# jnsquire/sregex

Measured on AMD Instinct MI355X. Metric: GB/s input scanned (whole job), gen-data stream resident in HBM, higher is better.
Workload: dtype u8; 1 GPU; configs[1]: /[a-z]+@[a-z]+\.[a-z]+/ Pike first-match + captures; 1 stream x 4.00 GiB gen-data (abccc.. + 'aaabbccb'); bytes_per_gpu=4294967293, streams_per_gpu=1, segment_bytes=16896, fixup_rounds=0, matches=0, engine=scan, lineage_passes=0, world_size=1

## Files before the change

### sregex_amd/csrc/sre_hip_batch.cpp

```cpp
#include <sregex_hip.h>
#include "sre_hip_runtime.h"
#include "sre_hip_scan.h"
#include "sre_scan_host.h"
#include "sre_dfa.h"
#include "sre_nfa.h"
#include "sre_hip_nfa.h"
#include "sre_nfa_wide.h"
#include "sre_hip_nfa_wide.h"
#include "sre_pwave.h"
#include "sre_hip_lines.h"
#include "sre_lines_gather.h"
#include "sre_lines_route.h"
#include "sre_lines_route_key.h"
#include "sre_lines_sort.h"
#include "sre_lines_sort_text.h"
#include "sre_lines_tally.h"
#include "sre_lines_tally_top.h"
#include "sre_lines_distinct.h"
#include "sre_lines_sums.h"
#include "sre_lines_keyset.h"
#include "sre_lines_join.h"
#include "sre_hip_streams.h"
#include "sre_streams_nfa.h"
#include <stddef.h>
#include <stdio.h>
#include <stdlib.h>
#include <string.h>
#include <atomic>
#include <chrono>
#include <initializer_list>
#include <vector>

#define SRE_SPECULATIVE_FIXUPS 2

struct sre_hip_scanner_s {
    sre_program_t     *prog;
    sre_hip_program_s *dp;
    int                mode, engine;
    char               kernel_name[64];
    uint32_t           ovec_slots;
    size_t             cap_streams;
    const void       **d_ptrs;
    uint64_t          *d_lens;
    int64_t           *d_records;
    void              *d_ctx;
    size_t             ctx_stride, ctx_cap;
    uint64_t          *h_lens;
    const void       **h_ptrs;
    size_t             last_n;
    hipStream_t        last_stream;
    sre_dfa_t                *dfa;
    sre_scan_device_tables_t *tab;
    uint32_t                  seg_override;
    uint64_t                  seg_cap_env;
    sre_scan_geom_t           geom;
    uint64_t                 *d_seg_first, *h_seg_first;
    sre_seg_summary_t        *d_sum;
    sre_seg_digest_t         *d_digest;
    size_t                    sum_cap;
    sre_stream_status_t      *d_status, *h_status;
    void                     *d_acc;
    int64_t                  *d_lo, *h_lo;
    uint16_t                 *d_scratch;
    size_t                    scratch_cap;
    sre_seg_lineage_t        *d_maps, *d_blocks;
    size_t                    maps_cap;
    uint8_t                  *d_fn;
    size_t                    fn_cap;
    int                       exact_passes;
    int                       lineage_passes;
    uint32_t                  next_init_variant;
    int                       blocks_per_cu;
    hipStream_t               tail_stream;
    bool                      tail_stream_set;
    int                       fixup_rounds;
    hipEvent_t                ev0, ev1;
    int                       ev_valid;
    sre_int_t                *h_records;
    hipEvent_t                ev_done;
    uint64_t                 *d_in, *h_in;
    unsigned char            *d_out, *h_out;
    sre_nfa_t                *nfa;
    sre_nfa_tables_t          ntab;
    sre_nfa_sa_tables_t       satab;
    bool                      use_sa;
    sre_nfa_wide_t           *wnfa;
    sre_nfa_wide_tables_t     wtab;
    uint64_t                 *d_wsets;
    bool                      wide_kernel;
    struct NfaCount          *cnt;
    uint8_t                  *d_sflags, *h_sflags;
    sre_nfa_count_req_t      *d_creq, *h_creq;
    size_t                    cnt_cap;
    int                       count_rounds;
    sre_pwave_hdr_t          *h_pwave;
    void                     *d_pwave;
    size_t                    layout_n;
    sre_nfa_summary_t        *d_nsum;
    size_t                    nsum_cap;
    uint64_t                 *d_belief;
    uint8_t                  *d_bvalid;
    uint64_t                 *d_nmat;
    size_t                    nmat_cap;
    void                     *d_nacc;
    sre_nfa_status_t         *d_nstatus, *h_nstatus;
    const uint64_t           *d_eset;
    uint64_t                 *d_ends;
    size_t                    ends_cap;
    uint64_t                 *d_lblk;
    size_t                    lblk_cap;
    int64_t                  *d_rows;
    size_t                    rows_cap;
    sre_lines_info_t         *d_linfo, *h_linfo;
    bool                      last_lines;
    int                       line_batches;
    double                    lines_kernel_ms;
    bool                      lines_device;
    size_t                    short_lines;
    hipEvent_t                ev_l0, ev_l1;
    uint64_t                 *d_fval;
    size_t                    fval_cap;
    uint64_t                 *d_fblk;
    size_t                    fblk_cap;
    uint64_t                 *d_cbits;
    size_t                    cbits_cap;
    uint64_t                 *d_cblk;
    size_t                    cblk_cap;
    uint64_t                 *d_fstart;
    size_t                    fstart_cap;
    uint8_t                  *d_lit;
    uint8_t                  *h_lit;
    size_t                    lit_len;
    bool                      lit_valid;
    uint64_t                 *d_rcnt;
    size_t                    rcnt_cap;
    uint64_t                 *d_rval;
    size_t                    rval_cap;
    uint64_t                 *d_rmeta;
    size_t                    rmeta_cap;
    int32_t                  *d_rmap;
    int32_t                  *h_rmap;
    bool                      rmap_valid;
    uint64_t                 *d_rres, *h_rres;
    uint64_t                 *d_ttab;
    size_t                    ttab_cap;
    uint32_t                 *d_tslot;
    size_t                    tslot_cap;
    uint64_t                 *d_vval;
    size_t                    vval_cap;
    uint64_t                 *d_vstart;
    size_t                    vstart_cap;
    sre_ls_agg_t             *d_vcopy;
    size_t                    vcopy_cap;
    int64_t                  *d_jkey;
    size_t                    jkey_cap;
    uint64_t                 *d_kitem[2];
    size_t                    kitem_cap[2];
    int8_t                   *d_sclass;
    size_t                    sclass_cap;
    uint32_t                 *d_sline[2];
    size_t                    sline_cap[2];
    uint64_t                 *d_pcount;
    size_t                    pcount_cap;
    sre_ls_agg_t             *d_psums;
    size_t                    psums_cap;
    uint64_t                 *d_pfirst;
    size_t                    pfirst_cap;
    uint32_t                 *d_pinv;
    size_t                    pinv_cap;
    uint64_t                 *d_pstart;
    size_t                    pstart_cap;
};

struct NfaCountStream {
    const uint8_t *base;
    uint64_t       n;
    uint64_t       cur;
    uint64_t       q;
    uint64_t       horizon;
    uint32_t       var_cur, var_q, mode_q;
    int64_t        count;
    bool           done, error;
    std::vector<sre_int_t> last;
};
struct NfaCount {
    std::vector<NfaCountStream> st;
    std::vector<size_t>         active;
};

static void
scanner_release(void *data)
{
    sre_hip_scanner_t *sc = static_cast<sre_hip_scanner_t *>(data);
    delete sc->cnt;
    free(sc->h_pwave);
    if (sc->d_pwave) (void) hipFree(sc->d_pwave);
    if (sc->d_sflags) (void) hipFree(sc->d_sflags);
    if (sc->h_sflags) (void) hipHostFree(sc->h_sflags);
    if (sc->d_creq) (void) hipFree(sc->d_creq);
    if (sc->h_creq) (void) hipHostFree(sc->h_creq);
    if (sc->d_in) (void) hipFree(sc->d_in);
    if (sc->h_in) (void) hipHostFree(sc->h_in);
    if (sc->d_out) (void) hipFree(sc->d_out);
    if (sc->h_out) (void) hipHostFree(sc->h_out);
    if (sc->d_ctx) (void) hipFree(sc->d_ctx);
    if (sc->d_sum) (void) hipFree(sc->d_sum);
    if (sc->d_digest) (void) hipFree(sc->d_digest);
    if (sc->d_acc) (void) hipFree(sc->d_acc);
    if (sc->d_lo) (void) hipFree(sc->d_lo);
    if (sc->h_lo) (void) hipHostFree(sc->h_lo);
    if (sc->d_scratch) (void) hipFree(sc->d_scratch);
    if (sc->d_fn) (void) hipFree(sc->d_fn);
    if (sc->d_maps) (void) hipFree(sc->d_maps);
    if (sc->d_blocks) (void) hipFree(sc->d_blocks);
    if (sc->ev0) (void) hipEventDestroy(sc->ev0);
    if (sc->ev1) (void) hipEventDestroy(sc->ev1);
    if (sc->ev_done) (void) hipEventDestroy(sc->ev_done);
    if (sc->ev_l0) (void) hipEventDestroy(sc->ev_l0);
    if (sc->ev_l1) (void) hipEventDestroy(sc->ev_l1);
    if (sc->d_nsum) (void) hipFree(sc->d_nsum);
    if (sc->d_belief) (void) hipFree(sc->d_belief);
    if (sc->d_bvalid) (void) hipFree(sc->d_bvalid);
    if (sc->d_nmat) (void) hipFree(sc->d_nmat);
    if (sc->d_nacc) (void) hipFree(sc->d_nacc);
    if (sc->d_ends) (void) hipFree(sc->d_ends);
    if (sc->d_lblk) (void) hipFree(sc->d_lblk);
    if (sc->d_rows) (void) hipFree(sc->d_rows);
    if (sc->d_fval) (void) hipFree(sc->d_fval);
    if (sc->d_fblk) (void) hipFree(sc->d_fblk);
    if (sc->d_cbits) (void) hipFree(sc->d_cbits);
    if (sc->d_cblk) (void) hipFree(sc->d_cblk);
    if (sc->d_fstart) (void) hipFree(sc->d_fstart);
    if (sc->d_lit) (void) hipFree(sc->d_lit);
    free(sc->h_lit);
    if (sc->d_rcnt) (void) hipFree(sc->d_rcnt);
    if (sc->d_rval) (void) hipFree(sc->d_rval);
    if (sc->d_rmeta) (void) hipFree(sc->d_rmeta);
    if (sc->d_rmap) (void) hipFree(sc->d_rmap);
    free(sc->h_rmap);
    if (sc->d_rres) (void) hipFree(sc->d_rres);
    if (sc->h_rres) (void) hipHostFree(sc->h_rres);
    if (sc->d_ttab) (void) hipFree(sc->d_ttab);
    if (sc->d_tslot) (void) hipFree(sc->d_tslot);
    if (sc->d_vval) (void) hipFree(sc->d_vval);
    if (sc->d_vstart) (void) hipFree(sc->d_vstart);
    if (sc->d_vcopy) (void) hipFree(sc->d_vcopy);
    if (sc->d_jkey) (void) hipFree(sc->d_jkey);
    if (sc->d_kitem[0]) (void) hipFree(sc->d_kitem[0]);
    if (sc->d_kitem[1]) (void) hipFree(sc->d_kitem[1]);
    if (sc->d_sclass) (void) hipFree(sc->d_sclass);
    if (sc->d_sline[0]) (void) hipFree(sc->d_sline[0]);
    if (sc->d_sline[1]) (void) hipFree(sc->d_sline[1]);
    if (sc->d_pcount) (void) hipFree(sc->d_pcount);
    if (sc->d_psums) (void) hipFree(sc->d_psums);
    if (sc->d_pfirst) (void) hipFree(sc->d_pfirst);
    if (sc->d_pinv) (void) hipFree(sc->d_pinv);
    if (sc->d_pstart) (void) hipFree(sc->d_pstart);
    if (sc->d_linfo) (void) hipFree(sc->d_linfo);
    if (sc->h_linfo) (void) hipHostFree(sc->h_linfo);
    if (sc->ntab.accept) (void) hipFree(const_cast<uint64_t *>(sc->ntab.accept));
    if (sc->ntab.follow) (void) hipFree(const_cast<uint64_t *>(sc->ntab.follow));
    if (sc->ntab.expand) (void) hipFree(const_cast<uint64_t *>(sc->ntab.expand));
    if (sc->ntab.kind) (void) hipFree(const_cast<uint8_t *>(sc->ntab.kind));
    if (sc->satab.accept) (void) hipFree(const_cast<uint64_t *>(sc->satab.accept));
    if (sc->satab.lut) (void) hipFree(const_cast<uint64_t *>(sc->satab.lut));
    if (sc->satab.expand) (void) hipFree(const_cast<uint64_t *>(sc->satab.expand));
    if (sc->d_wsets) (void) hipFree(sc->d_wsets);
    if (sc->wtab.accept) (void) hipFree(const_cast<uint64_t *>(sc->wtab.accept));
    if (sc->wtab.lut) (void) hipFree(const_cast<uint64_t *>(sc->wtab.lut));
    if (sc->wtab.expand) (void) hipFree(const_cast<uint64_t *>(sc->wtab.expand));
    if (sc->wtab.kind) (void) hipFree(const_cast<uint8_t *>(sc->wtab.kind));
    sre_nfa_wide_free(sc->wnfa);
    sre_nfa_free(sc->nfa);
    sre_scan_tables_release(sc->tab);
    sre_dfa_free(sc->dfa);
    free(sc);
}

static int
nfa_upload(sre_hip_scanner_t *sc)
{
    const sre_nfa_t *n = sc->nfa;
    const uint32_t   ns = n->nslices;
    std::vector<uint64_t> fol((size_t) ns * 256, 0), exp(16 * 256, 0);
    memcpy(fol.data(), n->follow.data(), n->follow.size() * sizeof(uint64_t));
    if (n->nassert) memcpy(exp.data(), n->expand.data(), exp.size() * sizeof(uint64_t));
    uint64_t *d_acc = NULL, *d_fol = NULL, *d_exp = NULL;
    uint8_t  *d_kind = NULL;
    SRE_HIP_TRY(hipMalloc(reinterpret_cast<void **>(&d_acc), 256 * sizeof(uint64_t)));
    sc->ntab.accept = d_acc;
// ... 360 lines not shown
sre_hip_scanner_kernel_name(sre_hip_scanner_t *sc)
{
    if (sc->kernel_name[0] == 0) {
        if (sc->engine == SRE_HIP_ENGINE_SCAN) {
            snprintf(sc->kernel_name, sizeof(sc->kernel_name), "sre_k_scan<%d, %d, %s, %s>",
                     sc->mode == SRE_HIP_PIKE_COUNT ? 2 : 1, (int) sc->tab->h.class_bits,
                     sc->tab->h.wide ? "true" : "false",
                     sc->mode == SRE_HIP_PIKE_COUNT && sc->tab->h.any_fresh ? "true" : "false");
        } else if (sc->engine == SRE_HIP_ENGINE_NFA) {
            if (sc->wide_kernel) sre_nfa_wide_kernel_name(&sc->wtab, sc->kernel_name, sizeof(sc->kernel_name));
            else if (sc->use_sa) sre_nfa_sa_kernel_name(&sc->satab, sc->kernel_name, sizeof(sc->kernel_name));
            else sre_nfa_kernel_name(sc->mode == SRE_HIP_THOMPSON ? 0 : 1, sc->ntab.nslices, sc->ntab.nassert != 0,
                                     sc->kernel_name, sizeof(sc->kernel_name));
        } else {
            snprintf(sc->kernel_name, sizeof(sc->kernel_name), "%s",
                     sc->mode == SRE_HIP_THOMPSON ? (sc->dp->has_wave ? "sre_k_thompson_wave_scan" : "sre_k_thompson_scan")
                                                  : sc->d_pwave ? "sre_k_pike_scan_wave" : "sre_k_pike_scan");
        }
    }
    return sc->kernel_name;
}

extern "C" SRE_API int
sre_hip_scanner_last_lineage_passes(sre_hip_scanner_t *sc)
{
    return sc->lineage_passes;
}

extern "C" SRE_API double
sre_hip_scanner_last_kernel_ms(sre_hip_scanner_t *sc)
{
    float ms = 0.0f;
    if (sc->last_lines) return sc->lines_kernel_ms;
    if (!sc->ev_valid) return -1.0;
    if (hipEventSynchronize(sc->ev1) != hipSuccess) return -1.0;
    if (hipEventElapsedTime(&ms, sc->ev0, sc->ev1) != hipSuccess) return -1.0;
    return (double) ms;
}

extern "C" SRE_API int
sre_hip_scanner_order_after_scan(sre_hip_scanner_t *sc, void *hip_stream)
{
    if (!sc->ev_valid) return 0;
    hipError_t e = hipStreamWaitEvent(static_cast<hipStream_t>(hip_stream), sc->ev1, 0);
    return e == hipSuccess ? 0 : sre_hip_fail("hipStreamWaitEvent", e);
}

extern "C" SRE_API int
sre_hip_scanner_set_tail_stream(sre_hip_scanner_t *sc, void *hip_stream)
{
    sc->tail_stream = static_cast<hipStream_t>(hip_stream);
    sc->tail_stream_set = hip_stream != NULL;
    return 0;
}

extern "C" SRE_API size_t
sre_hip_scanner_last_segment_bytes(sre_hip_scanner_t *sc)
{
    return sc->engine != SRE_HIP_ENGINE_VM ? sc->geom.seg_bytes : 0;
}

static size_t
record_bytes(const sre_hip_scanner_t *sc, size_t n)
{
    return n * (2 + (size_t) sc->ovec_slots) * sizeof(int64_t);
}

static int
scanner_reserve(sre_hip_scanner_t *sc, size_t n)
{
    if (n > sc->cap_streams) {
        if (sc->d_in) (void) hipFree(sc->d_in);
        if (sc->h_in) (void) hipHostFree(sc->h_in);
        if (sc->d_out) (void) hipFree(sc->d_out);
        if (sc->h_out) (void) hipHostFree(sc->h_out);
        if (sc->d_acc) (void) hipFree(sc->d_acc);
        if (sc->d_lo) (void) hipFree(sc->d_lo);
        if (sc->h_lo) (void) hipHostFree(sc->h_lo);
        sc->d_in = sc->h_in = NULL;
        sc->d_out = sc->h_out = NULL;
        sc->d_acc = NULL;
        sc->d_lo = sc->h_lo = NULL;
        sc->cap_streams = 0;
        const size_t in_bytes = (3 * n + 1) * sizeof(uint64_t);
        const size_t out_bytes = record_bytes(sc, n) + n * sizeof(sre_stream_status_t);
        static_assert(sizeof(sre_nfa_status_t) <= sizeof(sre_stream_status_t), "status block");
        static_assert(sizeof(sre_nfa_status_t) == sizeof(sre_nfa_window_t), "window layout");
        SRE_HIP_TRY(hipMalloc(reinterpret_cast<void **>(&sc->d_in), in_bytes));
        SRE_HIP_TRY(hipHostMalloc(reinterpret_cast<void **>(&sc->h_in), in_bytes, 0));
        SRE_HIP_TRY(hipMalloc(reinterpret_cast<void **>(&sc->d_out), out_bytes));
        SRE_HIP_TRY(hipHostMalloc(reinterpret_cast<void **>(&sc->h_out), out_bytes, 0));
        SRE_HIP_TRY(hipMalloc(&sc->d_acc, sre_scan_verify_acc_bytes((uint32_t) n)));
        SRE_HIP_TRY(sre_scan_verify_acc_init(sc->d_acc, (uint32_t) n, NULL));
        if (sc->engine == SRE_HIP_ENGINE_NFA) {
            if (sc->d_nacc) (void) hipFree(sc->d_nacc);
            sc->d_nacc = NULL;
            SRE_HIP_TRY(hipMalloc(&sc->d_nacc, sre_nfa_verify_acc_bytes((uint32_t) n)));
            SRE_HIP_TRY(sre_nfa_verify_acc_init(sc->d_nacc, (uint32_t) n, NULL));
        }
        SRE_HIP_TRY(hipStreamSynchronize(NULL));
        SRE_HIP_TRY(hipMalloc(reinterpret_cast<void **>(&sc->d_lo), n * sizeof(int64_t)));
        SRE_HIP_TRY(hipHostMalloc(reinterpret_cast<void **>(&sc->h_lo), n * sizeof(int64_t), 0));
        sc->cap_streams = n;
    }
    sc->layout_n = n;
    sc->h_ptrs = reinterpret_cast<const void **>(sc->h_in);
    sc->h_lens = sc->h_in + n;
    sc->h_seg_first = sc->h_in + 2 * n;
    sc->d_ptrs = reinterpret_cast<const void **>(sc->d_in);
    sc->d_lens = sc->d_in + n;
    sc->d_seg_first = sc->d_in + 2 * n;
    sc->d_records = reinterpret_cast<sre_int_t *>(sc->d_out);
    sc->h_records = reinterpret_cast<sre_int_t *>(sc->h_out);
    sc->d_status = reinterpret_cast<sre_stream_status_t *>(sc->d_out + record_bytes(sc, n));
    sc->h_status = reinterpret_cast<sre_stream_status_t *>(sc->h_out + record_bytes(sc, n));
    sc->d_nstatus = reinterpret_cast<sre_nfa_status_t *>(sc->d_status);
    sc->h_nstatus = reinterpret_cast<sre_nfa_status_t *>(sc->h_status);
    if ((sc->engine == SRE_HIP_ENGINE_VM || (sc->engine == SRE_HIP_ENGINE_NFA && sc->mode != SRE_HIP_THOMPSON && sc->d_pwave == NULL))
        && n * sc->ctx_stride > sc->ctx_cap)
    {
        if (sc->d_ctx) (void) hipFree(sc->d_ctx);
        sc->d_ctx = NULL;
        sc->ctx_cap = 0;
        SRE_HIP_TRY(hipMalloc(&sc->d_ctx, n * sc->ctx_stride));
        sc->ctx_cap = n * sc->ctx_stride;
    }
    return 0;
hip_failed:
    return -1;
}

static uint64_t
scan_seg_knobs(sre_hip_scanner_t *sc)
{
    uint64_t seg = sc->seg_override;
    const char *e = getenv("SRE_HIP_SEG_BYTES");
    if (seg == 0 && e && atoi(e) > 0 && atoi(e) % 256 == 0) seg = (uint64_t) atoi(e);
    e = getenv("SRE_HIP_SEG_CAP");
    sc->seg_cap_env = e && atoi(e) > 0 ? (uint64_t) atoi(e) : 0;
    return seg;
}

static uint64_t
nfa_seg_knobs(sre_hip_scanner_t *sc)
{
    uint64_t seg = scan_seg_knobs(sc);
    const char *e = getenv("SRE_HIP_SEG_BYTES");
    if (seg == 0 && e && atoi(e) > 0 && atoi(e) % 64 == 0) seg = (uint64_t) atoi(e);
    return seg;
}

static uint64_t
scan_seg_cap(const sre_hip_scanner_t *sc)
{
    return sc->seg_cap_env ? sc->seg_cap_env : 40960;
}

static int
scan_events(sre_hip_scanner_t *sc)
{
    if (sc->ev0 == NULL) {
        SRE_HIP_TRY(hipEventCreate(&sc->ev0));
        SRE_HIP_TRY(hipEventCreate(&sc->ev1));
    }
    return 0;
hip_failed:
    return -1;
}

static void
call_begin(sre_hip_scanner_t *sc)
{
    sc->last_lines = false;
    sc->fixup_rounds = 0;
    sc->exact_passes = 0;
    sc->lineage_passes = 0;
    sc->ev_valid = 0;
}

static void
geom_clear(sre_hip_scanner_t *sc)
{
    sc->geom = sre_scan_geom_t();
    sc->d_eset = NULL;
}

static void
geom_device(sre_hip_scanner_t *sc, uint64_t n, uint64_t seg, uint64_t nsegs)
{
    geom_clear(sc);
    sc->geom.streams = reinterpret_cast<const uint8_t *const *>(sc->d_ptrs);
    sc->geom.lens = sc->d_lens;
    sc->geom.seg_first = sc->d_seg_first;
    sc->geom.nstreams = (uint32_t) n;
    sc->geom.seg_bytes = (uint32_t) seg;
    sc->geom.nsegs = nsegs;
}

static uint64_t
scan_resident(sre_hip_scanner_t *sc)
{
    if (sc->blocks_per_cu == 0) {
        sc->blocks_per_cu = sc->engine == SRE_HIP_ENGINE_NFA
                                ? (sc->wide_kernel ? sre_nfa_wide_blocks_per_cu(&sc->wtab)
                                   : sc->use_sa ? sre_nfa_sa_blocks_per_cu(&sc->satab)
                                              : sre_nfa_blocks_per_cu(sc->mode == SRE_HIP_THOMPSON ? 0 : 1, sc->ntab.nslices,
                                                                      sc->ntab.nassert != 0))
                                                             : sre_scan_blocks_per_cu(&sc->tab->h);
    }
    return (uint64_t) sre_hip_cu_count() * (uint64_t) sc->blocks_per_cu * SRE_SCAN_BLOCK;
}

static int scan_buffers(sre_hip_scanner_t *sc, size_t nstreams, uint64_t seg, uint64_t nsegs);

static int
nfa_buffers(sre_hip_scanner_t *sc, uint64_t nsegs)
{
    if (nsegs > sc->nsum_cap) {
        if (sc->d_nsum) (void) hipFree(sc->d_nsum);
        if (sc->d_belief) (void) hipFree(sc->d_belief);
        if (sc->d_bvalid) (void) hipFree(sc->d_bvalid);
        if (sc->d_wsets) (void) hipFree(sc->d_wsets);
        sc->d_nsum = NULL;
        sc->d_belief = NULL;
        sc->d_bvalid = NULL;
        sc->d_wsets = NULL;
        sc->nsum_cap = 0;
        SRE_HIP_TRY(hipMalloc(reinterpret_cast<void **>(&sc->d_nsum), nsegs * sizeof(sre_nfa_summary_t)));
        SRE_HIP_TRY(hipMalloc(reinterpret_cast<void **>(&sc->d_belief), nsegs * nfa_words(sc) * sizeof(uint64_t)));
        if (sc->wide_kernel) SRE_HIP_TRY(hipMalloc(reinterpret_cast<void **>(&sc->d_wsets), nsegs * 2 * nfa_words(sc) * sizeof(uint64_t)));
        SRE_HIP_TRY(hipMalloc(reinterpret_cast<void **>(&sc->d_bvalid), nsegs));
        sc->nsum_cap = nsegs;
    }
    return 0;
hip_failed:
    return -1;
}

static int
scan_geometry(sre_hip_scanner_t *sc, size_t nstreams, uint32_t init_variant, uint32_t flags, uint32_t entry_state)
{
    uint64_t total = 0;
    for (size_t i = 0; i < nstreams; i++) total += sc->h_lens[i];
    uint64_t seg = scan_seg_knobs(sc);
    if (seg == 0) {
        const uint64_t resident = scan_resident(sc);
        seg = sre_scan_auto_segment(total, resident, scan_seg_cap(sc));
    }
    uint64_t nsegs = 0;
    for (size_t i = 0; i < nstreams; i++) {
        sc->h_seg_first[i] = nsegs;
        uint64_t k = (sc->h_lens[i] + seg - 1) / seg;
        nsegs += k ? k : 1;
    }
    sc->h_seg_first[nstreams] = nsegs;
    geom_clear(sc);
    sc->geom.streams = reinterpret_cast<const uint8_t *const *>(sc->d_ptrs);
    sc->geom.lens = sc->d_lens;
    sc->geom.seg_first = sc->d_seg_first;
    sc->geom.nstreams = (uint32_t) nstreams;
    sc->geom.seg_bytes = (uint32_t) seg;
    sc->geom.nsegs = nsegs;
    sc->geom.init_variant = init_variant;
    sc->geom.entry_state = entry_state;
    sc->geom.one_ptr = static_cast<const uint8_t *>(sc->h_ptrs[0]);
    sc->geom.one_len = sc->h_lens[0];
    sc->geom.flags = flags | ((nstreams == 1 && sc->engine == SRE_HIP_ENGINE_SCAN) ? SRE_GEOM_ONE : 0u);

    if (sc->engine == SRE_HIP_ENGINE_NFA) return nfa_buffers(sc, nsegs);
    return scan_buffers(sc, nstreams, seg, nsegs);
}

static int
scan_buffers(sre_hip_scanner_t *sc, size_t nstreams, uint64_t seg, uint64_t nsegs)
{
    if (nsegs > sc->sum_cap) {
        if (sc->d_sum) (void) hipFree(sc->d_sum);
        sc->d_sum = NULL;
        sc->sum_cap = 0;
        SRE_HIP_TRY(hipMalloc(reinterpret_cast<void **>(&sc->d_sum), nsegs * sizeof(sre_seg_summary_t)));
        sc->sum_cap = nsegs;
    }
    sc->geom.digest = NULL;
    if (nsegs <= SRE_VERIFY_ONE_SEGS && sc->mode != SRE_HIP_PIKE_COUNT) {
        if (sc->d_digest == NULL
            && hipMalloc(reinterpret_cast<void **>(&sc->d_digest), SRE_VERIFY_ONE_SEGS * sizeof(sre_seg_digest_t)) != hipSuccess)
        {
            sc->d_digest = NULL;
        }
        sc->geom.digest = sc->d_digest;
    }
    {
        size_t need = nstreams * ((size_t) seg + 16);
        if (need > sc->scratch_cap) {
            if (sc->d_scratch) (void) hipFree(sc->d_scratch);
            sc->d_scratch = NULL;
            sc->scratch_cap = 0;
            SRE_HIP_TRY(hipMalloc(reinterpret_cast<void **>(&sc->d_scratch), need * sizeof(uint16_t)));
            sc->scratch_cap = need;
        }
    }
    return 0;
hip_failed:
    return -1;
}

static int
nfa_windows(sre_hip_scanner_t *sc, const int64_t *d_lo, const sre_nfa_count_req_t *d_creq, hipStream_t stream)
{
    const uint32_t n = sc->geom.nstreams;
    if (sc->d_pwave) {
        SRE_HIP_TRY(sre_launch_pike_window_wave(sc->d_pwave, sc->h_pwave, sc->d_ptrs, sc->d_lens, n, sc->d_records,
                                                sc->ovec_slots, reinterpret_cast<sre_nfa_window_t *>(sc->d_nstatus), d_lo,
                                                d_creq, stream));
    } else {
        SRE_HIP_TRY(sre_launch_pike_window(sc->dp->d_blob, sc->dp->blob_bytes, sc->d_ptrs, sc->d_lens, n, sc->d_ctx, sc->ctx_stride,
                                           sc->d_records, sc->ovec_slots,
                                           reinterpret_cast<sre_nfa_window_t *>(sc->d_nstatus), d_lo,
                                           d_creq, stream));
    }
    return 0;
hip_failed:
    return -1;
}

static int
nfa_finish(sre_hip_scanner_t *sc, const int64_t *d_lo, const sre_nfa_count_req_t *d_creq, hipStream_t stream)
{
    const int kmode = sc->mode == SRE_HIP_THOMPSON ? SRE_HIP_THOMPSON : SRE_HIP_PIKE_FIRST;
    if (sc->wide_kernel) {
        SRE_HIP_TRY(sre_launch_nfa_wide_verify(kmode, sc->wtab.W, sc->geom, sc->d_nsum, sc->d_wsets, sc->d_nacc, sc->d_nstatus,
                                               sc->d_belief, sc->d_bvalid, sc->d_records, sc->ovec_slots, d_lo, stream));
    } else {
        SRE_HIP_TRY(sre_launch_nfa_verify(kmode, sc->geom, sc->d_nsum, sc->d_nacc, sc->d_nstatus,
                                          sc->d_belief, sc->d_bvalid, sc->d_records, sc->ovec_slots, d_lo, stream));
    }
    if (sc->mode != SRE_HIP_THOMPSON) return nfa_windows(sc, d_lo, d_creq, stream);
    return 0;
hip_failed:
    return -1;
}

static uint64_t
count_horizon(uint64_t dflt)
{
    const char *e = getenv("SRE_HIP_COUNT_HORIZON");
    return e && atoll(e) > 0 ? (uint64_t) atoll(e) : dflt;
}

static int
nfa_enqueue_pass(sre_hip_scanner_t *sc, size_t nstreams, uint32_t init_variant, const uint8_t *d_sflags,
                 const sre_nfa_count_req_t *d_creq, hipStream_t stream)
{
    if (scan_geometry(sc, nstreams, init_variant, 0, 0) != 0) return -1;
    sc->geom.sflags = d_sflags;
    SRE_HIP_TRY(hipMemcpyAsync(sc->d_in, sc->h_in, (3 * sc->layout_n + 1) * sizeof(uint64_t),
                               hipMemcpyHostToDevice, stream));
    if (scan_events(sc) != 0) return -1;
    {
        const bool timed = !sc->ev_valid;
        if (timed) SRE_HIP_TRY(hipEventRecord(sc->ev0, stream));
        SRE_HIP_TRY(nfa_launch_scan(sc, NULL, NULL, NULL, stream));
        if (timed) SRE_HIP_TRY(hipEventRecord(sc->ev1, stream));
        sc->ev_valid = 1;
    }
    if (sc->tail_stream_set && sc->tail_stream != stream) {
        SRE_HIP_TRY(hipStreamWaitEvent(sc->tail_stream, sc->ev1, 0));
        stream = sc->tail_stream;
    }
    return nfa_finish(sc, NULL, d_creq, stream);
hip_failed:
    return -1;
}
// ... 142 lines not shown
        SRE_HIP_TRY(hipMemcpyAsync(sc->h_out, sc->d_out, record_bytes(sc, sc->layout_n) + sc->layout_n * sizeof(sre_stream_status_t),
                                   hipMemcpyDeviceToHost, stream));
        SRE_HIP_TRY(hipStreamSynchronize(stream));
        {
            bool settled = true;
            if (nfa_settle(sc, na, sc->d_creq, stream, &settled) != 0) goto hip_failed;
            if (!settled) {
                SRE_HIP_TRY(hipMemcpyAsync(sc->h_out, sc->d_out, record_bytes(sc, sc->layout_n) + sc->layout_n * sizeof(sre_stream_status_t),
                                           hipMemcpyDeviceToHost, stream));
                SRE_HIP_TRY(hipStreamSynchronize(stream));
            }
        }
        for (size_t j = 0; j < na; j++) {
            NfaCountStream         &t = c.st[c.active[j]];
            const sre_nfa_status_t &w = sc->h_nstatus[j];
            const sre_int_t        *rec = sc->h_records + j * slots;
            const bool              truncated = (sc->h_sflags[j] & SRE_SFLAG_NO_EOF) != 0;
            if (getenv("SRE_HIP_DEBUG_COUNT")) {
                fprintf(stderr, "[sregex-hip] count round %d stream %zu: cur %llu q %llu var %u/%u mode %u len %llu%s -> ev %lld clean %lld "
                                "cmode %x rec %lld (%lld, %lld)\n", sc->count_rounds, c.active[j], (unsigned long long) t.cur,
                        (unsigned long long) t.q, t.var_cur, t.var_q, t.mode_q, (unsigned long long) sc->h_lens[j],
                        truncated ? " (truncated)" : "", (long long) w.ev_pos, (long long) w.clean_pos, w.clean_mode,
                        (long long) rec[0], (long long) rec[2], (long long) rec[3]);
            }
            if (w.ev_pos >= 0) {
                if (rec[0] < 0) {
                    fprintf(stderr, "[sregex-hip] find-all on the NFA tier: the exact window found no match behind an event\n");
                    t.error = t.done = true;
                    continue;
                }
                t.count++;
                t.last.assign(rec, rec + slots);
                const uint64_t end = (uint64_t) rec[3];
                const uint64_t gap = end > t.cur ? end - t.cur : 1;
                t.horizon = gap + gap / 4 < count_horizon(1u << 20) ? count_horizon(1u << 20) : gap + gap / 4;
                t.cur = t.q = end;
                t.var_cur = t.var_q = (w.clean_mode & SRE_NFA_MATCH_AFTER_NL) ? 1u : 2u;
                t.mode_q = 0;
                if (w.clean_mode & SRE_NFA_WINDOW_POISONED) t.error = t.done = true;
            } else if (!truncated) {
                t.done = true;
            } else if (w.clean_pos > 0) {
                t.q += (uint64_t) w.clean_pos;
                t.var_q = (w.clean_mode & SRE_NFA_CLEAN_AFTER_NL) ? 1u : 2u;
                t.mode_q = (uint32_t) (w.clean_mode & 1);
                t.horizon *= 2;
            } else {
                t.horizon *= 4;
            }
        }
    }
    sc->tail_stream_set = tail_set;
    for (size_t i = 0; i < n; i++) {
        const NfaCountStream &t = c.st[i];
        sre_int_t            *out = results + i * slots;
        if (t.count == 0) {
            out[0] = t.error ? SRE_ERROR : SRE_DECLINED;
            out[1] = 0;
            for (size_t k = 2; k < slots; k++) out[k] = -1;
        } else {
            for (size_t k = 0; k < slots; k++) out[k] = t.last[k];
            if (t.error) out[0] = SRE_ERROR;
            out[1] = (sre_int_t) t.count;
        }
    }
    return 0;
hip_failed:
    sc->tail_stream_set = tail_set;
    return -1;
}

extern "C" SRE_API int
sre_hip_scanner_last_count_rounds(sre_hip_scanner_t *sc)
{
    return sc->count_rounds;
}

extern "C" SRE_API int
sre_hip_scan_enqueue(sre_hip_scanner_t *sc, const void *const *d_streams, const size_t *lens,
    size_t nstreams, void *hip_stream)
{
    hipStream_t    stream = static_cast<hipStream_t>(hip_stream);
    const uint32_t init_variant = sc->next_init_variant;
    call_begin(sc);
    sc->next_init_variant = 0;
    if (nstreams == 0) {
        sc->last_n = 0;
        return 0;
    }
    if (scanner_reserve(sc, nstreams) != 0) return -1;
    for (size_t i = 0; i < nstreams; i++) {
        sc->h_ptrs[i] = d_streams[i];
        sc->h_lens[i] = lens[i];
    }
    if (sc->engine == SRE_HIP_ENGINE_VM) {
        SRE_HIP_TRY(hipMemcpyAsync(sc->d_in, sc->h_in, 2 * nstreams * sizeof(uint64_t),
                                   hipMemcpyHostToDevice, stream));
        if (sc->d_pwave && nstreams <= 16384) {
            SRE_HIP_TRY(sre_launch_pike_scan_wave(sc->d_pwave, sc->h_pwave, sc->mode, sc->d_ptrs, sc->d_lens,
                                                  (uint32_t) nstreams, sc->d_records, sc->ovec_slots, stream));
        } else {
            SRE_HIP_TRY(hipMemsetAsync(sc->d_ctx, 0, nstreams * sc->ctx_stride, stream));
            SRE_HIP_TRY(sre_launch_vm_scan(sc->dp->d_blob, sc->mode, sc->d_ptrs, sc->d_lens,
                                           (uint32_t) nstreams, sc->d_ctx, sc->ctx_stride,
                                           sc->d_records, sc->ovec_slots, sc->dp->has_wave, stream));
        }
    } else if (sc->engine == SRE_HIP_ENGINE_NFA && sc->cnt != NULL) {
        NfaCount &c = *sc->cnt;
        c.st.assign(nstreams, NfaCountStream());
        for (size_t i = 0; i < nstreams; i++) {
            NfaCountStream &t = c.st[i];
            t.base = static_cast<const uint8_t *>(d_streams[i]);
            t.n = lens[i];
            t.cur = t.q = 0;
            t.horizon = count_horizon(8u << 20);
            t.var_cur = t.var_q = init_variant;
            t.mode_q = 0;
            t.count = 0;
            t.done = t.error = false;
        }
        sc->count_rounds = 0;
        sc->last_n = nstreams;
        sc->last_stream = stream;
        return 0;
    } else if (sc->engine == SRE_HIP_ENGINE_NFA) {
        if (nfa_enqueue_pass(sc, nstreams, init_variant, NULL, NULL, stream) != 0) return -1;
        if (sc->tail_stream_set && sc->tail_stream != stream) stream = sc->tail_stream;
    } else {
        if (scan_geometry(sc, nstreams, init_variant, 0, 0) != 0) return -1;
        const bool one = (sc->geom.flags & SRE_GEOM_ONE) != 0;
        if (!one) {
            static const bool dma = getenv("SRE_HIP_DMA_UPLOAD") != NULL;
            if (dma) {
                SRE_HIP_TRY(hipMemcpyAsync(sc->d_in, sc->h_in, (3 * nstreams + 1) * sizeof(uint64_t),
                                           hipMemcpyHostToDevice, stream));
            } else {
                SRE_HIP_TRY(sre_launch_upload_words(sc->h_in, sc->d_in, (uint32_t) (3 * nstreams + 1), stream));
            }
        }
        if (scan_events(sc) != 0) return -1;
        SRE_HIP_TRY(hipEventRecord(sc->ev0, stream));
        SRE_HIP_TRY(sre_launch_scan(sc->tab->d_tab, sc->tab->h, sc->geom, sc->d_sum, NULL, NULL, stream));
        SRE_HIP_TRY(hipEventRecord(sc->ev1, stream));
        sc->ev_valid = 1;
        if (sc->tail_stream_set && sc->tail_stream != stream) {
            SRE_HIP_TRY(hipStreamWaitEvent(sc->tail_stream, sc->ev1, 0));
            stream = sc->tail_stream;
        }
        {
            const int fused = one && sc->geom.nsegs <= SRE_VERIFY_ONE_SEGS && sc->mode != SRE_HIP_PIKE_COUNT;
            if (!fused) SRE_HIP_TRY(sre_launch_verify(sc->tab->h, sc->geom, sc->d_sum, sc->d_acc, sc->d_status, stream));
            SRE_HIP_TRY(sre_launch_captures(sc->tab->d_tab, sc->tab->h, sc->geom, sc->d_sum, sc->d_status,
                                            sc->d_scratch, sc->d_records, sc->ovec_slots,
                                            NULL, NULL, 0, fused, stream));
        }
    }
    SRE_HIP_TRY(hipMemcpyAsync(sc->h_out, sc->d_out,
                               record_bytes(sc, nstreams)
                                   + (sc->engine != SRE_HIP_ENGINE_VM ? nstreams * sizeof(sre_stream_status_t) : 0),
                               hipMemcpyDeviceToHost, stream));
    if (sc->ev_done == NULL) SRE_HIP_TRY(hipEventCreateWithFlags(&sc->ev_done, hipEventDisableTiming));
    SRE_HIP_TRY(hipEventRecord(sc->ev_done, stream));
    sc->last_n = nstreams;
    sc->last_stream = stream;
    return 0;
hip_failed:
    return -1;
}

typedef uint64_t sre_lines_info_t::*LinfoWord;
#define LINFO(word) (&sre_lines_info_t::word)

static hipError_t
linfo_read(sre_hip_scanner_t *sc, hipStream_t stream, std::initializer_list<LinfoWord> words)
{
    const char *base = reinterpret_cast<const char *>(sc->h_linfo);
    size_t      lo = sizeof(sre_lines_info_t), hi = 0;
    for (LinfoWord w : words) {
        const size_t at = (size_t) (reinterpret_cast<const char *>(&(sc->h_linfo->*w)) - base);
        lo = at < lo ? at : lo;
        hi = at + sizeof(uint64_t) > hi ? at + sizeof(uint64_t) : hi;
    }
    return hipMemcpyAsync(reinterpret_cast<char *>(sc->h_linfo) + lo, reinterpret_cast<const char *>(sc->d_linfo) + lo, hi - lo,
                          hipMemcpyDeviceToHost, stream);
}

static int
lines_status_counters(sre_hip_scanner_t *sc, size_t n, hipStream_t stream)
{
    SRE_HIP_TRY(sre_launch_lines_settle(sc->d_status, (uint32_t) n, sc->d_linfo, stream));
    SRE_HIP_TRY(linfo_read(sc, stream, {LINFO(pending), LINFO(maps)}));
    SRE_HIP_TRY(hipStreamSynchronize(stream));
    return 0;
hip_failed:
    return -1;
}

static int
scan_settle(sre_hip_scanner_t *sc, size_t n, hipStream_t stream, bool with_captures, bool *psettled,
            bool counters = false)
{
    bool settled = true;
    int  batch = sc->mode == SRE_HIP_PIKE_COUNT ? 2 : SRE_SPECULATIVE_FIXUPS + 1;
    for (;;) {
        size_t pending = 0;
        if (counters) pending = (size_t) sc->h_linfo->pending;
        else for (size_t i = 0; i < n; i++) pending += sc->h_status[i].done ? 0 : 1;
        if (pending == 0) break;
        settled = false;
        for (int r = 0; r < batch; r++) {
            if (++sc->fixup_rounds > 1000000) {
                fprintf(stderr, "[sregex-hip] scanner fix-up did not converge\n");
                return -1;
            }
            const uint8_t *d_entry = NULL;
            static const bool count_exact = getenv("SRE_HIP_NO_COUNT_EXACT") == NULL;
            if ((sc->mode != SRE_HIP_PIKE_COUNT || count_exact) && sc->fixup_rounds > SRE_SPECULATIVE_FIXUPS) {
                if (sc->geom.nsegs > sc->fn_cap) {
                    if (sc->d_fn) (void) hipFree(sc->d_fn);
                    sc->d_fn = NULL;
                    sc->fn_cap = 0;
                    const size_t nchunks = sc->geom.nsegs / 256 + 1;
                    SRE_HIP_TRY(hipMalloc(reinterpret_cast<void **>(&sc->d_fn),
                                          sc->geom.nsegs * 64 + nchunks * 64 + nchunks + sc->geom.nsegs + 64));
                    sc->fn_cap = sc->geom.nsegs;
                }
                const size_t nchunks = sc->geom.nsegs / 256 + 1;
                uint8_t *d_comp = sc->d_fn + sc->geom.nsegs * 64, *d_chunk = d_comp + nchunks * 64;
                uint8_t *d_ent = d_chunk + nchunks;
                SRE_HIP_TRY(sre_launch_exact_entries(sc->tab->d_tab, sc->tab->h, sc->geom, sc->d_sum, sc->d_status,
                                                     sc->d_fn, d_comp, d_chunk, d_ent, stream));
                d_entry = d_ent;
                sc->exact_passes++;
            }
            SRE_HIP_TRY(sre_launch_scan(sc->tab->d_tab, sc->tab->h, sc->geom, sc->d_sum, sc->d_status, d_entry, stream));
            SRE_HIP_TRY(sre_launch_verify(sc->tab->h, sc->geom, sc->d_sum, sc->d_acc, sc->d_status, stream));
            if (with_captures) {
                SRE_HIP_TRY(sre_launch_captures(sc->tab->d_tab, sc->tab->h, sc->geom, sc->d_sum,
                                                sc->d_status, sc->d_scratch, sc->d_records,
                                                sc->ovec_slots, NULL, NULL, 0, 0, stream));
            }
        }
        if (counters) {
            if (lines_status_counters(sc, n, stream) != 0) return -1;
        } else {
            SRE_HIP_TRY(hipMemcpyAsync(sc->h_status, sc->d_status, n * sizeof(sre_stream_status_t),
                                       hipMemcpyDeviceToHost, stream));
            SRE_HIP_TRY(hipStreamSynchronize(stream));
        }
        batch = sc->mode == SRE_HIP_PIKE_COUNT ? (batch < 16 ? 2 * batch : 16) : 1;
    }
    if (psettled) *psettled = settled;
    return 0;
hip_failed:
    return -1;
}

static int
scan_lineage_pass(sre_hip_scanner_t *sc, hipStream_t stream)
{
    if (sc->geom.nsegs > sc->maps_cap) {
        if (sc->d_maps) (void) hipFree(sc->d_maps);
        if (sc->d_blocks) (void) hipFree(sc->d_blocks);
        sc->d_maps = sc->d_blocks = NULL;
        sc->maps_cap = 0;
        SRE_HIP_TRY(hipMalloc(reinterpret_cast<void **>(&sc->d_maps),
                              sc->geom.nsegs * sizeof(sre_seg_lineage_t)));
        SRE_HIP_TRY(hipMalloc(reinterpret_cast<void **>(&sc->d_blocks),
                              (sc->geom.nsegs / SRE_LINEAGE_BLOCK + 1) * sizeof(sre_seg_lineage_t)));
        sc->maps_cap = sc->geom.nsegs;
    }
    sc->lineage_passes++;
    SRE_HIP_TRY(sre_launch_lineage(sc->tab->d_tab, sc->tab->h, sc->geom, sc->d_sum,
                                   sc->d_status, sc->d_maps, sc->d_blocks, stream));
    SRE_HIP_TRY(sre_launch_captures(sc->tab->d_tab, sc->tab->h, sc->geom, sc->d_sum,
                                    sc->d_status, sc->d_scratch, sc->d_records,
                                    sc->ovec_slots, sc->d_maps, sc->d_blocks,
                                    1, 0, stream));
    return 0;
hip_failed:
    return -1;
}

extern "C" SRE_API int
sre_hip_scan_results(sre_hip_scanner_t *sc, sre_int_t *results)
{
    if (sc->last_lines) return -1;
    if (sc->last_n == 0) return 0;
    const size_t n = sc->last_n;
    hipStream_t  stream = sc->last_stream;

    const size_t bytes = n * (2 + (size_t) sc->ovec_slots) * sizeof(int64_t);
    bool         settled = true;

    if (sc->engine == SRE_HIP_ENGINE_NFA && sc->cnt != NULL) return nfa_count_rounds(sc, results);
    SRE_HIP_TRY(hipEventSynchronize(sc->ev_done));
    if (sc->engine == SRE_HIP_ENGINE_NFA && nfa_settle(sc, n, NULL, stream, &settled) != 0) return -1;
    if (sc->engine == SRE_HIP_ENGINE_SCAN) {
        if (scan_settle(sc, n, stream, true, &settled) != 0) return -1;
        if (sc->mode != SRE_HIP_THOMPSON) {
            size_t want = 0;
            for (size_t i = 0; i < n; i++) want += sc->h_status[i].need_maps != 0;
            if (want) {
                settled = false;
                if (scan_lineage_pass(sc, stream) != 0) return -1;
            }
        }
    }
    if (sc->engine == SRE_HIP_ENGINE_SCAN && getenv("SRE_HIP_DEBUG_STATUS")) {
        for (size_t i = 0; i < n && i < 8; i++) {
            const sre_stream_status_t &t = sc->h_status[i];
            fprintf(stderr, "[sregex-hip] stream %zu: rc %lld count %lld ev_pos %lld ev_sp %lld ev_state %u ev_sym %u "
                            "ev_apos %lld ev_astate %u ev_seg %lld limit %lld need_maps %d seg %u\n",
                    i, (long long) t.rc, (long long) t.count, (long long) t.ev_pos, (long long) t.ev_sp,
                    t.ev_state, t.ev_sym, (long long) t.ev_apos, t.ev_astate, (long long) t.ev_seg,
                    (long long) t.limit, t.need_maps, sc->geom.seg_bytes);
        }
        const size_t ns = sc->geom.nsegs < 16 ? (size_t) sc->geom.nsegs : 16;
        std::vector<sre_seg_summary_t> hs(ns);
// ... 159 lines not shown
    return 0;
hip_failed:
    return -1;
}

struct LinesTotals {
    int    fixups, exact, lineage;
    double kms;
    size_t nshort;
};

static int
lines_device_begin(sre_hip_scanner_t *sc, uint64_t rcap, size_t width, hipStream_t stream)
{
    if (rcap && lines_grow(&sc->d_rows, &sc->rows_cap, rcap * width * sizeof(int64_t)) != 0) return -1;
    SRE_HIP_TRY(hipMemsetAsync(&sc->d_linfo->reported, 0, sizeof(uint64_t), stream));
    return scan_events(sc);
hip_failed:
    return -1;
}

static int
lines_device_batch_end(sre_hip_scanner_t *sc, LinesTotals *tot, const LinesSink *sink, uint64_t nmax, uint64_t i0, int all,
                       uint64_t rcap, hipStream_t stream)
{
    const uint32_t slots = 2 + sc->ovec_slots;
    if (sink) {
        if (sink_select(sc, sink, slots, nmax, i0, stream) != 0) return -1;
    } else {
        SRE_HIP_TRY(sre_launch_lines_compact(sc->d_records, slots, nmax, i0, all, sc->d_ends, sc->d_lblk, sc->d_linfo, sc->d_rows,
                                             rcap, stream));
    }
    tot->fixups += sc->fixup_rounds;
    tot->exact += sc->exact_passes;
    tot->lineage += sc->lineage_passes;
    sc->line_batches++;
    return 0;
hip_failed:
    return -1;
}

static int
lines_device_end(sre_hip_scanner_t *sc, const LinesSink *sink, uint64_t n, sre_int_t *out, uint64_t rcap, size_t width,
                 uint64_t *pnrep, hipStream_t stream)
{
    if (sink) return 0;
    SRE_HIP_TRY(hipMemcpyAsync(&sc->h_linfo->reported, &sc->d_linfo->reported, sizeof(uint64_t), hipMemcpyDeviceToHost,
                               stream));
    SRE_HIP_TRY(hipStreamSynchronize(stream));
    *pnrep = n ? sc->h_linfo->reported : 0;
    {
        const uint64_t take = *pnrep < rcap ? *pnrep : rcap;
        if (take) {
            SRE_HIP_TRY(hipMemcpyAsync(out, sc->d_rows, take * width * sizeof(int64_t), hipMemcpyDeviceToHost, stream));
            SRE_HIP_TRY(hipStreamSynchronize(stream));
        }
    }
    return 0;
hip_failed:
    return -1;
}

static int
lines_scan_device(sre_hip_scanner_t *sc, const void *d_buf, uint64_t n, int all, sre_int_t *out, size_t cap,
                  uint64_t *pnrep, hipStream_t stream, LinesTotals *tot, const LinesSink *sink)
{
    const size_t   width = 3 + 2 + (size_t) sc->ovec_slots;
    const uint64_t bmax = lines_batch_limit();
    const uint64_t rcap = cap < n ? cap : n;
    const uint64_t seg_fixed = scan_seg_knobs(sc);
    const uint64_t resident = scan_resident(sc);
    if (lines_device_begin(sc, rcap, width, stream) != 0) return -1;
    for (uint64_t i0 = 0; i0 < n;) {
        const uint64_t nmax = bmax < n - i0 ? bmax : n - i0;
        if (scanner_reserve(sc, nmax) != 0) return -1;
        SRE_HIP_TRY(sre_launch_lines_geometry(d_buf, sc->d_ends, n, i0, nmax, SRE_LINES_WALK_MAX, seg_fixed, resident,
                                              scan_seg_cap(sc), reinterpret_cast<const uint8_t **>(sc->d_ptrs), sc->d_lens,
                                              sc->d_seg_first, sc->d_lblk, sc->d_linfo, stream));
        SRE_HIP_TRY(linfo_read(sc, stream, {LINFO(i1), LINFO(seg), LINFO(nsegs)}));
        SRE_HIP_TRY(hipStreamSynchronize(stream));
        const uint64_t i1 = sc->h_linfo->i1, nb = i1 - i0, seg = sc->h_linfo->seg, nsegs = sc->h_linfo->nsegs;
        call_begin(sc);
        geom_device(sc, nb, seg, nsegs);
        if (scan_buffers(sc, nb, seg, nsegs) != 0) return -1;
        SRE_HIP_TRY(hipEventRecord(sc->ev0, stream));
        SRE_HIP_TRY(sre_launch_scan(sc->tab->d_tab, sc->tab->h, sc->geom, sc->d_sum, NULL, NULL, stream));
        SRE_HIP_TRY(hipEventRecord(sc->ev1, stream));
        SRE_HIP_TRY(sre_launch_verify(sc->tab->h, sc->geom, sc->d_sum, sc->d_acc, sc->d_status, stream));
        SRE_HIP_TRY(sre_launch_captures(sc->tab->d_tab, sc->tab->h, sc->geom, sc->d_sum, sc->d_status,
                                        sc->d_scratch, sc->d_records, sc->ovec_slots, NULL, NULL, 0, 0, stream));
        if (lines_status_counters(sc, nb, stream) != 0) return -1;
        if (scan_settle(sc, nb, stream, true, NULL, true) != 0) return -1;
        if (sc->mode != SRE_HIP_THOMPSON && sc->h_linfo->maps != 0 && scan_lineage_pass(sc, stream) != 0) return -1;
        if (lines_device_batch_end(sc, tot, sink, nmax, i0, all, rcap, stream) != 0) return -1;
        {
            float ms = 0.0f;
            SRE_HIP_TRY(hipEventElapsedTime(&ms, sc->ev0, sc->ev1));
            tot->kms += ms;
        }
        i0 = i1;
    }
    return lines_device_end(sc, sink, n, out, rcap, width, pnrep, stream);
hip_failed:
    return -1;
}

static uint64_t
lines_short_max(const sre_hip_scanner_t *sc)
{
    if (sc->wide_kernel) return 0;
    const char *e = getenv("SRE_HIP_LINES_SHORT_MAX");
    if (e == NULL || *e == 0) return SRE_LINES_SHORT_MAX;
    const long long v = atoll(e);
    return v <= 0 ? 0 : v < (1ll << 20) ? (uint64_t) v : (uint64_t) 1 << 20;
}

static int
lines_scan_nfa(sre_hip_scanner_t *sc, const void *d_buf, uint64_t n, int all, sre_int_t *out, size_t cap,
               uint64_t *pnrep, hipStream_t stream, LinesTotals *tot, const LinesSink *sink)
{
    const size_t   width = 3 + 2 + (size_t) sc->ovec_slots;
    const uint64_t rcap = cap < n ? cap : n;
    const uint64_t lmax = lines_short_max(sc), short_lim = lmax ? lmax + 1 : 0;
    const uint32_t W = nfa_words(sc);
    const uint64_t seg_cost = sizeof(sre_nfa_summary_t) + W * sizeof(uint64_t) + 1 + (sc->wide_kernel ? 2 * W * sizeof(uint64_t) : 0);
    uint64_t       bmax = lines_batch_limit();
    const uint64_t seg_fixed = nfa_seg_knobs(sc);
    const uint64_t resident = scan_resident(sc);
    if (sc->mode != SRE_HIP_THOMPSON && sc->d_pwave == NULL && sc->ctx_stride) {
        const uint64_t most = SRE_LINES_NFA_WORK_MAX / sc->ctx_stride;
        if (bmax > most) bmax = most ? most : 1;
    }
    sre_lnfa_t ltab;
    memset(&ltab, 0, sizeof(ltab));
    if (short_lim) ltab = sc->use_sa ? sre_lines_nfa_tables_sa(&sc->satab) : sre_lines_nfa_tables_plain(&sc->ntab);
    if (lines_device_begin(sc, rcap, width, stream) != 0) return -1;
    if (sc->ev_l0 == NULL) {
        SRE_HIP_TRY(hipEventCreate(&sc->ev_l0));
        SRE_HIP_TRY(hipEventCreate(&sc->ev_l1));
    }
    for (uint64_t i0 = 0; i0 < n;) {
        const uint64_t nmax = bmax < n - i0 ? bmax : n - i0;
        if (scanner_reserve(sc, nmax) != 0) return -1;
        SRE_HIP_TRY(sre_launch_lines_geometry_nfa(d_buf, sc->d_ends, n, i0, nmax, short_lim, SRE_LINES_NFA_WORK_MAX, seg_cost,
                                                  seg_fixed, resident, scan_seg_cap(sc), reinterpret_cast<const uint8_t **>(sc->d_ptrs),
                                                  sc->d_lens, sc->d_seg_first, sc->d_lblk, sc->d_linfo, stream));
        SRE_HIP_TRY(linfo_read(sc, stream, {LINFO(i1), LINFO(seg), LINFO(nsegs)}));
        SRE_HIP_TRY(hipMemcpyAsync(&sc->h_linfo->nshort, &sc->d_linfo->nshort, sizeof(uint64_t), hipMemcpyDeviceToHost, stream));
        SRE_HIP_TRY(hipStreamSynchronize(stream));
        const uint64_t i1 = sc->h_linfo->i1, nb = i1 - i0, seg = sc->h_linfo->seg, nsegs = sc->h_linfo->nsegs;
        const uint64_t nshort = sc->h_linfo->nshort;
        call_begin(sc);
        geom_device(sc, nb, seg, nsegs);
        if (nsegs) {
            if (nfa_buffers(sc, nsegs) != 0) return -1;
            SRE_HIP_TRY(hipEventRecord(sc->ev0, stream));
            SRE_HIP_TRY(nfa_launch_scan(sc, NULL, NULL, NULL, stream));
            SRE_HIP_TRY(hipEventRecord(sc->ev1, stream));
            if (nfa_finish(sc, NULL, NULL, stream) != 0) return -1;
        }
        if (nshort) {
            SRE_HIP_TRY(hipEventRecord(sc->ev_l0, stream));
            SRE_HIP_TRY(sre_launch_lines_nfa(ltab, d_buf, sc->d_ends, i0, (uint32_t) nb, (uint32_t) short_lim,
                                             sc->mode == SRE_HIP_THOMPSON, sc->d_nstatus, sc->d_records, sc->ovec_slots, sc->d_lo,
                                             stream));
            SRE_HIP_TRY(hipEventRecord(sc->ev_l1, stream));
            if (sc->mode != SRE_HIP_THOMPSON && nfa_windows(sc, sc->d_lo, NULL, stream) != 0) return -1;
        }
        if (nsegs && nfa_settle_device(sc, nb, stream) != 0) return -1;
        if (lines_device_batch_end(sc, tot, sink, nmax, i0, all, rcap, stream) != 0) return -1;
        {
// ... 1438 lines not shown
            res.need_bytes = (size_t) sc->h_linfo->fneed;
            res.nwritten = (size_t) nwritten;
            res.out_bytes = (size_t) out_bytes;
            res.passes = passes;
            res.vmin = vmin;
            res.vmax = vmax;
            SRE_HIP_TRY(sre_launch_extract_gather(d_buf, d_out, sc->d_rval, sc->d_pstart, nrows * k, out_bytes, (uint32_t) delim,
                                                  (uint32_t) fsep, stream));
            const uint64_t counts_rows = counts_cap < nrows ? counts_cap : nrows, sums_rows = sums_cap < nrows ? sums_cap : nrows;
            const uint64_t index_rows = index_cap < nwritten ? index_cap : nwritten;
            SRE_HIP_TRY(sre_launch_tally_top_permute(keys, nkeys, nrows, sc->d_pcount, psums, v, sc->d_pfirst, sc->d_ends, n, sc->d_pstart,
                                                     sc->d_rval, k, sc->d_jkey, sc->d_sclass, d_counts, counts_rows, d_sums, sums_rows,
                                                     reinterpret_cast<int64_t *>(d_index), index_rows, sc->d_pinv, stream));
        }
        SRE_HIP_TRY(sre_launch_tally_top_ranks(sc->d_tslot, t.cnt, sc->d_pinv, rank_cap < n ? rank_cap : n, nkeys,
                                               reinterpret_cast<int64_t *>(d_rank), stream));
        SRE_HIP_TRY(hipStreamSynchronize(stream));
    }
    if (info) *info = res;
    return rc;
hip_failed:
    return -1;
}

extern "C" SRE_API int
sre_hip_scanner_last_line_batches(sre_hip_scanner_t *sc)
{
    return sc->line_batches;
}

extern "C" SRE_API int
sre_hip_scanner_last_lines_device(sre_hip_scanner_t *sc)
{
    return sc->lines_device ? 1 : 0;
}

extern "C" SRE_API size_t
sre_hip_scanner_last_short_lines(sre_hip_scanner_t *sc)
{
    return sc->short_lines;
}

extern "C" int
sre_hip_scan_one(sre_hip_scanner_t *sc, const void *d_buf, size_t len, int init_variant,
    sre_int_t *rec, int *poisoned, hipStream_t stream)
{
    const void *ptrs[1] = {d_buf};
    size_t      lens[1] = {len};
    sc->next_init_variant = (uint32_t) init_variant;
    if (sre_hip_scan_enqueue(sc, ptrs, lens, 1, stream) != 0) return -1;
    if (sre_hip_scan_results(sc, rec) != 0) return -1;
    if (poisoned) {
        *poisoned = sc->engine == SRE_HIP_ENGINE_SCAN ? sc->h_status[0].error
                  : sc->engine == SRE_HIP_ENGINE_NFA ? (sc->h_nstatus[0].clean_mode & SRE_NFA_WINDOW_POISONED) != 0 : 0;
    }
    return 0;
}

extern "C" int
sre_hip_scan_stream_chunk(sre_hip_scanner_t *sc, const void *d_buf, size_t len, int init_variant,
    int continues, uint32_t entry_state, int eof, int64_t base, sre_stream_ctx_t *d_ctx,
    sre_stream_result_t *d_res, const sre_stream_result_t *h_res, uint32_t ovec_slots, hipStream_t stream,
    void (*midway)(void *), void *midway_arg)
{
    struct Midway {
        void (*fn)(void *);
        void  *arg;
        void   run() { if (fn) fn(arg); fn = nullptr; }
        ~Midway() { run(); }
    } mid{midway, midway_arg};
    if (sc->engine != SRE_HIP_ENGINE_SCAN || sc->mode == SRE_HIP_PIKE_COUNT) return -1;
    call_begin(sc);
    if (scanner_reserve(sc, 1) != 0) return -1;
    sc->h_ptrs[0] = d_buf;
    sc->h_lens[0] = len;
    if (scan_geometry(sc, 1, (uint32_t) init_variant, (continues ? SRE_GEOM_CONTINUES : 0u) | (eof ? 0u : SRE_GEOM_NO_EOF),
                      entry_state) != 0)
    {
        return -1;
    }
    SRE_HIP_TRY(sre_launch_scan(sc->tab->d_tab, sc->tab->h, sc->geom, sc->d_sum, NULL, NULL, stream));
    {
        const int fused = sc->geom.nsegs <= SRE_VERIFY_ONE_SEGS;
        if (!fused) SRE_HIP_TRY(sre_launch_verify(sc->tab->h, sc->geom, sc->d_sum, sc->d_acc, sc->d_status, stream));
        SRE_HIP_TRY(sre_launch_stream_tail(sc->tab->d_tab, sc->tab->h, sc->geom, sc->d_sum, sc->d_status,
                                           sc->d_scratch, d_ctx, d_res, base, eof, ovec_slots, fused, stream));
    }
    mid.run();
    {
        const volatile int64_t *prc = &h_res->rc;
        const auto              t0 = std::chrono::steady_clock::now();
        const auto              limit = std::chrono::microseconds(200 + (int64_t) (len >> 12));
        while (*prc == SRE_STREAM_PENDING) {
            if (std::chrono::steady_clock::now() - t0 > limit) {
                SRE_HIP_TRY(hipStreamSynchronize(stream));
                break;
            }
        }
        std::atomic_thread_fence(std::memory_order_acquire);
    }
    if (h_res->rc == SRE_STREAM_UNSETTLED) {
        SRE_HIP_TRY(hipMemcpyAsync(sc->h_status, sc->d_status, sizeof(sre_stream_status_t),
                                   hipMemcpyDeviceToHost, stream));
        SRE_HIP_TRY(hipStreamSynchronize(stream));
        if (scan_settle(sc, 1, stream, false, NULL) != 0) return -1;
        SRE_HIP_TRY(sre_launch_stream_tail(sc->tab->d_tab, sc->tab->h, sc->geom, sc->d_sum, sc->d_status,
                                           sc->d_scratch, d_ctx, d_res, base, eof, ovec_slots, 0, stream));
        SRE_HIP_TRY(hipStreamSynchronize(stream));
    }
    sc->last_n = 0;
    return 0;
hip_failed:
    return -1;
}

extern "C" int
sre_hip_scanner_streams(sre_hip_scanner_t *sc)
{
    if (sc->engine != SRE_HIP_ENGINE_SCAN) return 0;
    if (sc->mode == SRE_HIP_THOMPSON) return 1;
    return sc->mode == SRE_HIP_PIKE_FIRST && sc->tab->h.max_threads <= SRE_STREAM_MAX_THREADS
           && sc->tab->h.nslots <= SRE_STREAM_MAX_SLOTS;
}


struct sre_hip_streams_s {
    sre_hip_scanner_t    *sc;
    size_t                n;
    sre_streams_layout_t  L;
    int64_t              *d_rows;
    size_t                rows_bytes;
    uint8_t              *d_rekind;
    sre_streams_feed_t   *d_feed, *h_feed;
    uint32_t             *d_sentry;
    unsigned char        *d_out, *h_out;
    sre_stream_result_t  *d_tailres;
    uint64_t             *d_idx;
    size_t                idx_cap;
    int                   fixups, launches;
    int                   engine;
    uint32_t              W;
    sre_streams_nfa_init_t init0;
    uint64_t             *d_eset;
    uint8_t              *d_sflags;
    int                   exact_passes;
};

static sre_hip_streams_t *streams_create_on(sre_pool_t *pool, sre_hip_scanner_t *sc, int mode, size_t nstreams);

static void
streams_release(void *data)
{
    sre_hip_streams_t *ss = static_cast<sre_hip_streams_t *>(data);
    if (ss->d_rows) (void) hipFree(ss->d_rows);
    if (ss->d_rekind) (void) hipFree(ss->d_rekind);
    if (ss->d_feed) (void) hipFree(ss->d_feed);
    if (ss->h_feed) (void) hipHostFree(ss->h_feed);
    if (ss->d_sentry) (void) hipFree(ss->d_sentry);
    if (ss->d_out) (void) hipFree(ss->d_out);
    if (ss->h_out) (void) hipHostFree(ss->h_out);
    if (ss->d_tailres) (void) hipFree(ss->d_tailres);
    if (ss->d_idx) (void) hipFree(ss->d_idx);
    if (ss->d_eset) (void) hipFree(ss->d_eset);
    if (ss->d_sflags) (void) hipFree(ss->d_sflags);
    free(ss);
}

// ... 189 lines not shown
        SRE_HIP_TRY(sre_launch_streams_nfa_prologue(ss->d_feed, (uint32_t) n, ss->d_rows, ss->W, ss->init0, ss->L.rec_slots, seg_fixed,
                                                    resident, scan_seg_cap(sc),
                                                    reinterpret_cast<const uint8_t **>(sc->d_ptrs), sc->d_lens, sc->d_seg_first,
                                                    ss->d_sflags, ss->d_eset, d_recs, d_info, stream));
        SRE_HIP_TRY(hipMemcpyAsync(ss->h_out, ss->d_out, sizeof(sre_streams_info_t), hipMemcpyDeviceToHost, stream));
        SRE_HIP_TRY(hipStreamSynchronize(stream));
        ss->launches += 3;
    }
    if (h_info->nsegs != 0) {
        if (nfa_buffers(sc, h_info->nsegs) != 0) return -1;
        geom_device(sc, n, h_info->seg, h_info->nsegs);
        sc->geom.sflags = ss->d_sflags;
        sc->d_eset = ss->d_eset;
        SRE_HIP_TRY(nfa_launch_scan(sc, NULL, NULL, NULL, stream));
        if (nfa_finish(sc, NULL, NULL, stream) != 0) return -1;
        SRE_HIP_TRY(sre_launch_streams_nfa_tail(ss->d_feed, (uint32_t) n, ss->d_rows, ss->W, sc->d_seg_first, sc->d_nstatus, sc->d_nsum,
                                                sc->wide_kernel ? sc->d_wsets : NULL, ss->L.rec_slots, d_recs, d_info, 0, stream));
        ss->launches += 1 + 3 + 1;
    }
    SRE_HIP_TRY(hipMemcpyAsync(ss->h_out, ss->d_out, out_bytes, hipMemcpyDeviceToHost, stream));
    SRE_HIP_TRY(hipStreamSynchronize(stream));
    ss->launches += 1;
    if (h_info->unsettled != 0) {
        if (nfa_settle_device(sc, n, stream) != 0) return -1;
        SRE_HIP_TRY(hipMemsetAsync(&d_info->unsettled, 0, sizeof(uint64_t), stream));
        SRE_HIP_TRY(sre_launch_streams_nfa_tail(ss->d_feed, (uint32_t) n, ss->d_rows, ss->W, sc->d_seg_first, sc->d_nstatus, sc->d_nsum,
                                                sc->wide_kernel ? sc->d_wsets : NULL, ss->L.rec_slots, d_recs, d_info, 1, stream));
        SRE_HIP_TRY(hipMemcpyAsync(ss->h_out, ss->d_out, out_bytes, hipMemcpyDeviceToHost, stream));
        SRE_HIP_TRY(hipStreamSynchronize(stream));
        ss->fixups = sc->fixup_rounds;
        ss->exact_passes = sc->exact_passes;
        ss->launches += 3;
        if (h_info->unsettled != 0) {
            fprintf(stderr, "[sregex-hip] stream set: %llu streams did not settle\n", (unsigned long long) h_info->unsettled);
            return -1;
        }
    }
    memcpy(results, ss->h_out + sizeof(sre_streams_info_t), n * ss->L.rec_slots * sizeof(int64_t));
    return 0;
hip_failed:
    return -1;
}

extern "C" SRE_API int
sre_hip_streams_feed(sre_hip_streams_t *ss, const void *const *d_chunks, const size_t *lens,
    const unsigned char *eof, sre_int_t *results, void *hip_stream)
{
    if (ss == NULL || d_chunks == NULL || lens == NULL || eof == NULL || results == NULL) return -1;
    hipStream_t         stream = static_cast<hipStream_t>(hip_stream);
    sre_hip_scanner_t  *sc = ss->sc;
    const size_t        n = ss->n;
    sre_streams_info_t *d_info = reinterpret_cast<sre_streams_info_t *>(ss->d_out);
    const volatile sre_streams_info_t *h_info = reinterpret_cast<sre_streams_info_t *>(ss->h_out);
    int64_t            *d_recs = reinterpret_cast<int64_t *>(ss->d_out + sizeof(sre_streams_info_t));
    const size_t        out_bytes = sizeof(sre_streams_info_t) + n * ss->L.rec_slots * sizeof(int64_t);
    ss->fixups = 0;
    ss->launches = 0;
    ss->exact_passes = 0;
    call_begin(sc);
    sc->last_n = 0;
    for (size_t i = 0; i < n; i++) {
        ss->h_feed[i].ptr = (uint64_t) reinterpret_cast<uintptr_t>(d_chunks[i]);
        ss->h_feed[i].len = d_chunks[i] ? lens[i] : 0;
        ss->h_feed[i].flags = d_chunks[i] ? (SRE_SFEED_FED | (eof[i] ? SRE_SFEED_EOF : 0u)) : 0u;
    }
    if (scanner_reserve(sc, n) != 0) return -1;
    if (ss->engine == SRE_HIP_ENGINE_NFA) return streams_feed_nfa(ss, results, stream);
    {
        const uint64_t seg_fixed = scan_seg_knobs(sc);
        const uint64_t resident = scan_resident(sc);
        SRE_HIP_TRY(sre_launch_upload_words(reinterpret_cast<const uint64_t *>(ss->h_feed),
                                            reinterpret_cast<uint64_t *>(ss->d_feed), (uint32_t) (3 * n), stream));
        SRE_HIP_TRY(sre_launch_streams_prologue(ss->d_feed, (uint32_t) n, ss->d_rows, ss->L, ss->d_rekind, sc->tab->h.init[0],
                                                seg_fixed, resident, scan_seg_cap(sc),
                                                reinterpret_cast<const uint8_t **>(sc->d_ptrs), sc->d_lens, sc->d_seg_first,
                                                ss->d_sentry, d_recs, d_info, stream));
        SRE_HIP_TRY(hipMemcpyAsync(ss->h_out, ss->d_out, sizeof(sre_streams_info_t), hipMemcpyDeviceToHost, stream));
        SRE_HIP_TRY(hipStreamSynchronize(stream));
        ss->launches += 3;
    }
    if (h_info->nsegs != 0) {
        const uint64_t seg = h_info->seg, nsegs = h_info->nsegs;
        const uint32_t grid = streams_tail_grid(h_info->nactive);
        if (scan_buffers(sc, grid, seg, nsegs) != 0) return -1;
        geom_device(sc, n, seg, nsegs);
        sc->geom.sentry = ss->d_sentry;
        SRE_HIP_TRY(sre_launch_scan(sc->tab->d_tab, sc->tab->h, sc->geom, sc->d_sum, NULL, NULL, stream));
        SRE_HIP_TRY(sre_launch_verify(sc->tab->h, sc->geom, sc->d_sum, sc->d_acc, sc->d_status, stream));
        SRE_HIP_TRY(sre_launch_streams_tail(sc->tab->d_tab, sc->tab->h, sc->geom, sc->d_sum, sc->d_status, sc->d_scratch,
                                            ss->d_rows, ss->L, ss->d_tailres, d_recs, d_info, grid, 0, stream));
        ss->launches += 1 + (sc->mode == SRE_HIP_PIKE_FIRST && sc->tab->h.nshadow ? 4 : 3) + 1;
    }
    SRE_HIP_TRY(hipMemcpyAsync(ss->h_out, ss->d_out, out_bytes, hipMemcpyDeviceToHost, stream));
    SRE_HIP_TRY(hipStreamSynchronize(stream));
    ss->launches += 1;
    if (h_info->unsettled != 0) {
        const uint32_t grid = streams_tail_grid(h_info->nactive);
        sc->h_linfo->pending = h_info->unsettled;
        sc->h_linfo->maps = 0;
        if (scan_settle(sc, n, stream, false, NULL, true) != 0) return -1;
        SRE_HIP_TRY(hipMemsetAsync(&d_info->unsettled, 0, sizeof(uint64_t), stream));
        SRE_HIP_TRY(sre_launch_streams_tail(sc->tab->d_tab, sc->tab->h, sc->geom, sc->d_sum, sc->d_status, sc->d_scratch,
                                            ss->d_rows, ss->L, ss->d_tailres, d_recs, d_info, grid, 1, stream));
        SRE_HIP_TRY(hipMemcpyAsync(ss->h_out, ss->d_out, out_bytes, hipMemcpyDeviceToHost, stream));
        SRE_HIP_TRY(hipStreamSynchronize(stream));
        ss->fixups = sc->fixup_rounds;
        ss->exact_passes = sc->exact_passes;
        ss->launches += 3;
        if (h_info->unsettled != 0) {
            fprintf(stderr, "[sregex-hip] stream set: %llu streams did not settle\n", (unsigned long long) h_info->unsettled);
            return -1;
        }
    }
    memcpy(results, ss->h_out + sizeof(sre_streams_info_t), n * ss->L.rec_slots * sizeof(int64_t));
    return 0;
hip_failed:
    return -1;
}


extern "C" SRE_API void *
sre_hip_alloc(size_t bytes)
{
    void *p = NULL;
    if (sre_hip_ready() != 0) return NULL;
    hipError_t e = hipMalloc(&p, bytes ? bytes : 1);
    if (e != hipSuccess) {
        sre_hip_fail("hipMalloc", e);
        return NULL;
    }
    return p;
}

extern "C" SRE_API void
sre_hip_free(void *d_ptr)
{
    if (d_ptr) (void) hipFree(d_ptr);
}

extern "C" SRE_API int
sre_hip_upload(void *d_dst, const void *h_src, size_t bytes)
{
    hipError_t e = hipMemcpy(d_dst, h_src, bytes, hipMemcpyHostToDevice);
    return e == hipSuccess ? 0 : sre_hip_fail("hipMemcpy H2D", e);
}

extern "C" SRE_API int
sre_hip_download(void *h_dst, const void *d_src, size_t bytes)
{
    hipError_t e = hipMemcpy(h_dst, d_src, bytes, hipMemcpyDeviceToHost);
    return e == hipSuccess ? 0 : sre_hip_fail("hipMemcpy D2H", e);
}

extern "C" SRE_API int
sre_hip_synchronize(void *hip_stream)
{
    hipError_t e = hipStreamSynchronize(static_cast<hipStream_t>(hip_stream));
    return e == hipSuccess ? 0 : sre_hip_fail("hipStreamSynchronize", e);
}

extern "C" SRE_API int
sre_hip_gen_data(void *d_dst, size_t n, const void *h_tail, size_t tail_len, void *hip_stream)
{
    hipStream_t stream = static_cast<hipStream_t>(hip_stream);
    void       *d_tail = NULL;
    int         rc = -1;
    if (sre_hip_ready() != 0 || tail_len > n) return -1;
    SRE_HIP_TRY(hipMalloc(&d_tail, tail_len ? tail_len : 1));
    if (tail_len) {
        SRE_HIP_TRY(hipMemcpyAsync(d_tail, h_tail, tail_len, hipMemcpyHostToDevice, stream));
    }
// ... 46 lines not shown
```

### sregex_amd/csrc/sre_hip_scan.h

```cpp
#ifndef SRE_HIP_SCAN_H
#define SRE_HIP_SCAN_H

#include <hip/hip_runtime.h>
#include <stdint.h>

#define SRE_CEILING_GRID   2048

#include "sre_scan_fast.h"

#define SRE_SCAN_MAX_SHADOWS  2u
#define SRE_SCAN_MAX_ROWS(bits)   ((65536u - 768u - ((bits) == 8 ? 512u : (8u / (bits)) * 512u)) / 1024u)
#define SRE_SCAN_MAX_STATES       62u
#define SRE_SCAN_BLOCK        256u
#define SRE_SCAN_LDS_LIMIT    (128u * 1024u)
#define SRE_CAPTURE_MAX_GRID   16384u
#define SRE_CAPTURE_LANE_STREAMS 4096u
#define SRE_CAPTURE_LDS_LIMIT  (144u * 1024u)
#define SRE_SCAN_ROUND        64u
#define SRE_SCAN_LINE         128u
#define SRE_SCAN_SEG_ALIGN    256u

#define SRE_SCAN_NINIT 4u
#define SRE_DEV_EV_DONE_EMPTY 3
#define SRE_DEV_EV_POP_FULL   4
// ... 62 lines not shown
} sre_seg_summary_t;

typedef struct sre_seg_digest_s {
    uint32_t s_in, s_out, bits, count;
} sre_seg_digest_t;

#define SRE_SUM_PENDING   1u
#define SRE_SUM_TERM      2u
#define SRE_SUM_LASTEV    4u
#define SRE_SUM_ERROR     8u
#define SRE_SUM_IN_PENDING 16u
#define SRE_SUM_STABLE    32u

#define SRE_STATE_SKIP    0x40000000u

typedef struct {
    uint64_t anc;
    uint16_t saved;
    uint16_t stop;
    uint32_t pad;
} sre_seg_lineage_t;

#define SRE_LINEAGE_BLOCK  256u
#define SRE_WALK_BUDGET    256

#define SRE_STREAM_MAX_THREADS 64u
#define SRE_STREAM_MAX_SLOTS   64u
typedef struct {
    uint32_t state;
    uint32_t has_pending;
    int64_t  pending_regex;
    int64_t  pending_vec[SRE_STREAM_MAX_SLOTS];
    int64_t  caps[SRE_STREAM_MAX_THREADS][SRE_STREAM_MAX_SLOTS];
    int64_t  caps_next[SRE_STREAM_MAX_THREADS][SRE_STREAM_MAX_SLOTS];
} sre_stream_ctx_t;

#define SRE_VERIFY_ONE_SEGS 8192u
#define SRE_STREAM_UNSETTLED (-100)
#define SRE_STREAM_PENDING   (-101)

typedef struct {
    int64_t  rc;
    int64_t  has_pending, pending[2];
    int64_t  ev_in_chunk;
    int64_t  poisoned;
    int64_t  next_state;
    int64_t  ev_slot1;
    int64_t  ov[SRE_STREAM_MAX_SLOTS];
} sre_stream_result_t;

typedef struct {
    int64_t  first_bad;
    int64_t  limit;
    int64_t  count;
    int64_t  rc;
    int64_t  ev_pos, ev_sp;
    uint32_t ev_state, ev_sym;
    int64_t  ev_apos;
    uint32_t ev_astate;
    uint32_t valid_from;
    int64_t  ev_seg;
    int64_t  unst_seg;
    int64_t  unst_end;
    int32_t  done;
    int32_t  error;
    int32_t  need_maps;
    int32_t  pad;
} sre_stream_status_t;

typedef struct {
    const uint8_t *const *streams;
    const uint64_t *lens;
    const uint64_t *seg_first;
    uint32_t nstreams;
    uint32_t seg_bytes;
    uint64_t nsegs;
    uint32_t init_variant;
    uint32_t flags;
    uint32_t entry_state;
    const uint8_t *one_ptr;
    uint64_t one_len;
    const uint8_t *sflags;
    struct sre_seg_digest_s *digest;
    const uint32_t *sentry;
} sre_scan_geom_t;
#define SRE_SENTRY_STATE(e)   ((e) & 0xffffu)
#define SRE_SENTRY_CONTINUES  0x40000000u
#define SRE_SENTRY_NO_EOF     0x80000000u
#define SRE_SFLAG_INIT(f)    ((f) & 3u)
#define SRE_SFLAG_SNAP(f)    (((f) >> 2) & 3u)
#define SRE_SFLAG_MODE(f)    (((f) >> 4) & 1u)
#define SRE_SFLAG_NO_EOF     32u

#define SRE_GEOM_CONTINUES 1u
#define SRE_GEOM_NO_EOF    2u
#define SRE_GEOM_ONE       4u

#ifdef __HIPCC__
static __host__ __device__ inline uint64_t
sre_scan_auto_segment(uint64_t total, uint64_t resident, uint64_t seg_cap)
{
    uint64_t rounds = (total + resident * seg_cap - 1) / (resident * seg_cap);
    if (rounds < 1) rounds = 1;
    const uint64_t lanes = resident * rounds - (resident * rounds >> 6);
    uint64_t       seg = (total / lanes + SRE_SCAN_SEG_ALIGN) / SRE_SCAN_SEG_ALIGN * SRE_SCAN_SEG_ALIGN;
    if (seg < 256) seg = 256;
    if (seg % 4096 == 0) seg += SRE_SCAN_SEG_ALIGN;
    return seg;
}

static __device__ inline const uint8_t *
geom_ptr(const sre_scan_geom_t &G, uint32_t s)
{
    return (G.flags & SRE_GEOM_ONE) ? G.one_ptr : G.streams[s];
}
static __device__ inline uint64_t
geom_len(const sre_scan_geom_t &G, uint32_t s)
{
    return (G.flags & SRE_GEOM_ONE) ? G.one_len : G.lens[s];
}
static __device__ inline uint64_t
geom_first(const sre_scan_geom_t &G, uint32_t i)
{
    return (G.flags & SRE_GEOM_ONE) ? (i ? G.nsegs : 0) : G.seg_first[i];
}
#endif

#ifdef __cplusplus
extern "C" {
#endif
hipError_t sre_launch_gen_data(void *d_dst, uint64_t n, uint64_t tail_len, const void *d_tail,
    hipStream_t stream);
hipError_t sre_launch_read_ceiling(const void *d_src, uint64_t n, uint32_t *d_sink,
    hipStream_t stream);
hipError_t sre_launch_read_pattern(const void *d_src, uint64_t n, uint32_t seg_bytes,
    uint32_t tile, uint32_t lds_bytes, uint32_t *d_sink, hipStream_t stream);

size_t sre_scan_lds_bytes(const sre_scan_tables_t *h_tab);
int sre_scan_blocks_per_cu(const sre_scan_tables_t *h_tab);

hipError_t sre_launch_scan(const sre_scan_tables_t *d_tab, sre_scan_tables_t h_tab,
    sre_scan_geom_t geom, sre_seg_summary_t *d_sum, const sre_stream_status_t *d_lo, const uint8_t *d_entry,
    hipStream_t stream);
hipError_t sre_launch_exact_entries(const sre_scan_tables_t *d_tab, sre_scan_tables_t h_tab,
    sre_scan_geom_t geom, const sre_seg_summary_t *d_sum, const sre_stream_status_t *d_status,
    uint8_t *d_fn, uint8_t *d_comp, uint8_t *d_chunk_entry, uint8_t *d_entry, hipStream_t stream);
hipError_t sre_launch_stream_tail(const sre_scan_tables_t *d_tab, sre_scan_tables_t h_tab,
    sre_scan_geom_t geom, const sre_seg_summary_t *d_sum, sre_stream_status_t *d_status,
    uint16_t *d_scratch, sre_stream_ctx_t *d_ctx, sre_stream_result_t *result, int64_t base, int eof,
    uint32_t ovec_slots, int verify, hipStream_t stream);
hipError_t sre_launch_upload_words(const uint64_t *h_src_mapped, uint64_t *d_dst, uint32_t nwords, hipStream_t stream);
size_t sre_scan_verify_acc_bytes(uint32_t nstreams);
hipError_t sre_scan_verify_acc_init(void *d_acc, uint32_t nstreams, hipStream_t stream);
hipError_t sre_launch_verify(sre_scan_tables_t h_tab, sre_scan_geom_t geom,
    const sre_seg_summary_t *d_sum, void *d_acc, sre_stream_status_t *d_status,
    hipStream_t stream);
hipError_t sre_launch_captures(const sre_scan_tables_t *d_tab, sre_scan_tables_t h_tab,
    sre_scan_geom_t geom, const sre_seg_summary_t *d_sum, sre_stream_status_t *d_status,
    uint16_t *d_scratch, int64_t *d_records, uint32_t ovec_slots,
    const sre_seg_lineage_t *d_maps, const sre_seg_lineage_t *d_blocks, int use_maps,
    int verify, hipStream_t stream);
hipError_t sre_launch_lineage(const sre_scan_tables_t *d_tab, sre_scan_tables_t h_tab,
    sre_scan_geom_t geom, const sre_seg_summary_t *d_sum, const sre_stream_status_t *d_status,
    sre_seg_lineage_t *d_maps, sre_seg_lineage_t *d_blocks, hipStream_t stream);
#ifdef __cplusplus
}
#endif
#endif
```

### sregex_amd/csrc/sre_hip_scan.hip

```cpp
#include <hip/hip_runtime.h>
#include <stdlib.h>
#include "sre_hip_scan.h"
#include "sre_hip_streams.h"
#include "sre_hip_tile.h"

#define SRE_HIP_PIKE_COUNT 2
#define EV_DONE 1
#define EV_POP  2
#define RC_DECLINED (-5)
#define RC_ERROR    (-1)


__global__ void
sre_k_gen_data(uint8_t *__restrict__ dst, uint64_t n, uint64_t body, const uint8_t *__restrict__ tail)
{
    const uint64_t stride = (uint64_t) gridDim.x * blockDim.x * 16;
    for (uint64_t base = ((uint64_t) blockIdx.x * blockDim.x + threadIdx.x) * 16; base < n;
         base += stride)
    {
        uint8_t  v[16];
        unsigned ph = (unsigned) (base % 5);
#pragma unroll
        for (int k = 0; k < 16; k++) {
            uint64_t i = base + k;
            uint8_t  c = ph == 0 ? 'a' : ph == 1 ? 'b' : 'c';
            if (i >= body && i < n) c = tail[i - body];
            v[k] = c;
            ph = ph == 4 ? 0 : ph + 1;
        }
        if (base + 16 <= n) {
            *reinterpret_cast<uint4 *>(dst + base) = *reinterpret_cast<uint4 *>(v);
        } else {
            for (int k = 0; k < 16 && base + k < n; k++) dst[base + k] = v[k];
        }
    }
}

extern "C" hipError_t
sre_launch_gen_data(void *d_dst, uint64_t n, uint64_t tail_len, const void *d_tail,
                    hipStream_t stream)
{
    if (n == 0) return hipSuccess;
    uint64_t lanes = (n + 15) / 16;
    uint32_t block = 256;
    uint64_t grid = (lanes + block - 1) / block;
    if (grid > 8192) grid = 8192;
    hipLaunchKernelGGL(sre_k_gen_data, dim3((uint32_t) grid), dim3(block), 0, stream,
                       static_cast<uint8_t *>(d_dst), n, n - tail_len,
                       static_cast<const uint8_t *>(d_tail));
    return hipGetLastError();
}


__global__ void
sre_k_read_ceiling(const uint4 *__restrict__ src, uint64_t nvec, uint32_t *__restrict__ sink)
{
    uint32_t       acc = 0;
    const uint64_t stride = (uint64_t) gridDim.x * blockDim.x;
    uint64_t       i = (uint64_t) blockIdx.x * blockDim.x + threadIdx.x;
    for (; i + 3 * stride < nvec; i += 4 * stride) {
        uint4 a = src[i], b = src[i + stride], c = src[i + 2 * stride], d = src[i + 3 * stride];
        acc += (a.x ^ a.y ^ a.z ^ a.w) + (b.x ^ b.y ^ b.z ^ b.w) + (c.x ^ c.y ^ c.z ^ c.w)
               + (d.x ^ d.y ^ d.z ^ d.w);
    }
    for (; i < nvec; i += stride) {
        uint4 a = src[i];
        acc += a.x ^ a.y ^ a.z ^ a.w;
    }
    if (acc == 0x9e3779b9u) sink[blockIdx.x] = acc;
}

extern "C" hipError_t
sre_launch_read_ceiling(const void *d_src, uint64_t n, uint32_t *d_sink, hipStream_t stream)
{
    uint64_t nvec = n / 16;
    if (nvec == 0) return hipSuccess;
    hipLaunchKernelGGL(sre_k_read_ceiling, dim3(SRE_CEILING_GRID), dim3(256), 0, stream,
                       static_cast<const uint4 *>(d_src), nvec, d_sink);
    return hipGetLastError();
}


template <int TILE>
__global__ __launch_bounds__(256) void
sre_k_read_pattern(const uint8_t *__restrict__ src, uint64_t n, uint32_t seg_bytes,
                   uint32_t *__restrict__ sink)
{
// ... 1037 lines not shown
                const int64_t e = pop ? pend : pend + 1;
                sp = empty ? e + 1 : e;
            } else if (++guard < 2) {
                sp = q;
            }
            if (pend >= 0) guard = 0;
            if (sp < 1) sp = 1;
            if (sp > n) sp = n;
            cur = tabp->init[restart_variant_of(*tabp, data[sp - 1])];
            pend = -1;
            q = sp - 1;
        }
    };
    for (; p + 16 <= seg_b; p += 16) {
        const sre_u32x4 v = *reinterpret_cast<const __attribute__((address_space(1))) sre_u32x4_unaligned *>(
            reinterpret_cast<uintptr_t>(data + p));
        const uint32_t words[4] = {v.x, v.y, v.z, v.w};
        uint32_t       t = fast_lds + cur * SRE_FAST_ROW_BYTES;
#pragma unroll
        for (int j = 0; j < GIDX; j++) {
            uint32_t ix = 0;
#pragma unroll
            for (int u = 0; u < STRIDE; u++) {
                const int      b = j * STRIDE + u;
                const uint32_t c = (words[b >> 2] >> ((b & 3) * 8)) & 0xffu;
                ix |= BITS == 8 ? c << 2 : (uint32_t) clsx[u][c];
            }
            t = *(lds_u32_t) (uintptr_t) ((t & 0xffffu) + ix);
        }
        if (t & LDS_SLOW) exact(p, p + 16);
        else cur = ((t & 0xffffu) - fast_lds) / SRE_FAST_ROW_BYTES;
    }
    exact(p, seg_b);
    fn[g * 64 + lane] = (uint8_t) cur;
}

__global__ __launch_bounds__(64) void
sre_k_fn_chunks(uint64_t nsegs, const uint8_t *__restrict__ fn, uint8_t *__restrict__ comp)
{
    const uint64_t c = blockIdx.x;
    uint32_t       v = threadIdx.x;
    const uint64_t g0 = c * SRE_FN_CHUNK, g1 = g0 + SRE_FN_CHUNK <= nsegs ? g0 + SRE_FN_CHUNK : nsegs;
    for (uint64_t g = g0; g < g1; g++) v = fn[g * 64 + (v & 63u)];
    comp[c * 64 + threadIdx.x] = (uint8_t) v;
}

__global__ void
sre_k_fn_resolve(sre_scan_geom_t G, const sre_seg_summary_t *__restrict__ sum,
                 const sre_stream_status_t *__restrict__ status, const uint8_t *__restrict__ fn,
                 const uint8_t *__restrict__ comp, uint8_t *__restrict__ entry, uint8_t *__restrict__ chunk_entry)
{
    const uint32_t s = blockIdx.x * blockDim.x + threadIdx.x;
    if (s >= G.nstreams || status[s].done || status[s].first_bad < 1) return;
    const uint64_t first = geom_first(G, s), g_hi = geom_first(G, s + 1);
    uint64_t       g = first + (uint64_t) status[s].first_bad;
    uint32_t       v = sum[g - 1].s_out & 63u;
    while (g < g_hi) {
        if (g % SRE_FN_CHUNK == 0 && g + SRE_FN_CHUNK <= g_hi) {
            chunk_entry[g / SRE_FN_CHUNK] = (uint8_t) v;
            v = comp[(g / SRE_FN_CHUNK) * 64 + v];
            g += SRE_FN_CHUNK;
        } else {
            entry[g] = (uint8_t) v;
            v = fn[g * 64 + v];
            g++;
        }
    }
}

__global__ void
sre_k_fn_fill(uint64_t nsegs, const uint8_t *__restrict__ fn, const uint8_t *__restrict__ chunk_entry,
              uint8_t *__restrict__ entry)
{
    const uint64_t c = (uint64_t) blockIdx.x * blockDim.x + threadIdx.x;
    if (c * SRE_FN_CHUNK >= nsegs || chunk_entry[c] == 0xffu) return;
    uint32_t v = chunk_entry[c];
    for (uint64_t g = c * SRE_FN_CHUNK; g < (c + 1) * SRE_FN_CHUNK && g < nsegs; g++) {
        entry[g] = (uint8_t) v;
        v = fn[g * 64 + (v & 63u)];
    }
}


struct VerifyAcc {
    unsigned long long bad, end;
    unsigned long long count, evseg, spseg;
    unsigned long long unst;
    unsigned long long unst_end;
};

__global__ __launch_bounds__(256) void
sre_k_verify_a(sre_scan_geom_t G, const sre_seg_summary_t *__restrict__ sum, VerifyAcc *__restrict__ acc,
               int mode)
{
    SRE_TAIL_PRIO();
    const uint64_t g = (uint64_t) blockIdx.x * blockDim.x + threadIdx.x;
    const bool     valid = g < G.nsegs;
    const uint32_t s = stream_of(G, valid ? g : G.nsegs - 1);
    unsigned long long kb = ~0ull, ke = ~0ull;
    if (valid) {
        const uint64_t k = g - geom_first(G, s);
        const uint32_t s_in = sum[g].s_in;
        bool           bad = s_in == 0xffffffffu;
        if (k > 0) {
            const sre_seg_summary_t &p = sum[g - 1], &c = sum[g];
            if (s_in != p.s_out) bad = true;
            if (mode == SRE_HIP_PIKE_COUNT) {
                const bool pp = (p.flags & SRE_SUM_PENDING) != 0, cp = (c.flags & SRE_SUM_IN_PENDING) != 0;
                if (pp != cp) bad = true;
                if (pp && cp && (p.pe_pos != c.in_pe_pos || p.pe_state != c.in_pe_state || p.pe_sym != c.in_pe_sym)) {
                    bad = true;
                }
            }
        }
        if (bad) kb = k;
        if (sum[g].flags & SRE_SUM_TERM) ke = k;
    }
    const uint32_t s0 = (uint32_t) __builtin_amdgcn_readfirstlane((int) s);
    if (__builtin_amdgcn_ballot_w64(s != s0) == 0) {
        for (int d = 32; d >= 1; d >>= 1) {
            const unsigned long long ob = __shfl_xor(kb, d, 64), oe = __shfl_xor(ke, d, 64);
            kb = ob < kb ? ob : kb;
            ke = oe < ke ? oe : ke;
        }
        if ((threadIdx.x & 63u) != 0) kb = ke = ~0ull;
    }
    if (kb != ~0ull && kb < __hip_atomic_load(&acc[s].bad, __ATOMIC_RELAXED, __HIP_MEMORY_SCOPE_AGENT)) atomicMin(&acc[s].bad, kb);
    if (ke != ~0ull && ke < __hip_atomic_load(&acc[s].end, __ATOMIC_RELAXED, __HIP_MEMORY_SCOPE_AGENT)) atomicMin(&acc[s].end, ke);
}

#define SRE_VERIFY_SPAN 1024u

__global__ __launch_bounds__(256) void
sre_k_verify_b(sre_scan_geom_t G, const sre_seg_summary_t *__restrict__ sum, VerifyAcc *__restrict__ acc)
{
    SRE_TAIL_PRIO();
    __shared__ unsigned long long sh_count, sh_ev, sh_sp;
    const uint64_t g0 = (uint64_t) blockIdx.x * SRE_VERIFY_SPAN;
    const uint64_t glast = (g0 + SRE_VERIFY_SPAN - 1 < G.nsegs) ? g0 + SRE_VERIFY_SPAN - 1 : G.nsegs - 1;
    const uint32_t s_first = stream_of(G, g0), s_last = stream_of(G, glast);
    const bool     uniform = (s_first == s_last);
    if (threadIdx.x == 0) {
        sh_count = 0;
        sh_ev = 0;
        sh_sp = 0;
    }
    __syncthreads();
    unsigned long long my_count = 0, my_ev = 0, my_sp = 0;
    for (uint32_t it = 0; it < SRE_VERIFY_SPAN / 256; it++) {
        const uint64_t g = g0 + it * 256u + threadIdx.x;
        if (g >= G.nsegs) break;
        const uint32_t s = uniform ? s_first : stream_of(G, g);
        const uint64_t k = g - geom_first(G, s);
        const uint64_t nseg = geom_first(G, s + 1) - geom_first(G, s);
        uint64_t       bad = acc[s].bad, end = acc[s].end;
        if (bad > nseg) bad = nseg;
        if (end > nseg) end = nseg;
        const uint64_t limit = end < bad ? end + 1 : bad;
        if (k < limit) {
            const sre_seg_summary_t &c = sum[g];
            if (uniform) {
                my_count += (unsigned long long) c.count;
                if (c.flags & SRE_SUM_LASTEV) my_ev = (unsigned long long) k + 1;
                if (c.cur_sp >= 0) my_sp = (unsigned long long) k + 1;
            } else {
                if (c.count) atomicAdd(&acc[s].count, (unsigned long long) c.count);
                if (c.flags & SRE_SUM_LASTEV) atomicMax(&acc[s].evseg, (unsigned long long) k + 1);
                if (c.cur_sp >= 0) atomicMax(&acc[s].spseg, (unsigned long long) k + 1);
            }
        }
    }
    if (uniform) {
        for (int d = 32; d >= 1; d >>= 1) {
            my_count += __shfl_down(my_count, d, 64);
            const unsigned long long e2 = __shfl_down(my_ev, d, 64), s2 = __shfl_down(my_sp, d, 64);
            my_ev = e2 > my_ev ? e2 : my_ev;
            my_sp = s2 > my_sp ? s2 : my_sp;
        }
        if ((threadIdx.x & 63u) == 0) {
            if (my_count) atomicAdd(&sh_count, my_count);
            if (my_ev) atomicMax(&sh_ev, my_ev);
            if (my_sp) atomicMax(&sh_sp, my_sp);
        }
    }
    __syncthreads();
    if (uniform && threadIdx.x == 0) {
        if (sh_count) atomicAdd(&acc[s_first].count, sh_count);
        if (sh_ev) atomicMax(&acc[s_first].evseg, sh_ev);
        if (sh_sp) atomicMax(&acc[s_first].spseg, sh_sp);
    }
}

__global__ __launch_bounds__(256) void
sre_k_verify_b2(sre_scan_geom_t G, const sre_seg_summary_t *__restrict__ sum, VerifyAcc *__restrict__ acc)
{
    SRE_TAIL_PRIO();
    __shared__ unsigned long long sh_max, sh_max_end;
    const uint64_t g0 = (uint64_t) blockIdx.x * SRE_VERIFY_SPAN;
    const uint64_t glast = (g0 + SRE_VERIFY_SPAN - 1 < G.nsegs) ? g0 + SRE_VERIFY_SPAN - 1 : G.nsegs - 1;
    const uint32_t s_first = stream_of(G, g0), s_last = stream_of(G, glast);
    const bool     uniform = (s_first == s_last);
    if (threadIdx.x == 0) sh_max = sh_max_end = 0;
    __syncthreads();
    unsigned long long mine = 0, mine_end = 0;
    for (uint32_t it = 0; it < SRE_VERIFY_SPAN / 256; it++) {
        const uint64_t g = g0 + it * 256u + threadIdx.x;
        if (g >= G.nsegs) break;
        const uint32_t s = uniform ? s_first : stream_of(G, g);
        const uint64_t k = g - geom_first(G, s);
        const uint64_t evseg = acc[s].evseg;
        const uint64_t nseg = geom_first(G, s + 1) - geom_first(G, s);
        if (!(sum[g].flags & SRE_SUM_STABLE)) {
            unsigned long long m1 = 0, m2 = 0;
            if (evseg != 0 && k + 1 < evseg) m1 = k + 1;
// ... 58 lines not shown
        const sre_seg_summary_t &c = sum[evseg - 1];
        st.ev_apos = c.lm_apos;
        st.ev_astate = c.lm_astate;
        st.ev_state = c.lm_state;
        st.ev_sym = c.lm_sym;
        st.ev_pos = c.lm_pos;
        st.ev_sp = c.lm_sp;
        st.ev_seg = (int64_t) evseg - 1;
        st.rc = T.trans[(size_t) c.lm_state * (T.ncls + 1) + c.lm_sym].regex;
        if (T.mode != SRE_HIP_PIKE_COUNT) st.count = 1;
        if (st.ev_sp < 0) {
            int64_t        sp = 0;
            const uint64_t spseg = acc.spseg;
            if (T.mode != SRE_HIP_PIKE_COUNT || spseg == 0) {
                sp = 0;
            } else if (spseg < evseg) {
                sp = sum[spseg - 1].cur_sp;
            } else if (defer_search) {
                sp = SRE_EV_SP_SEARCH;
            } else {
                for (int64_t q = (int64_t) evseg - 2; q >= 0; q--) {
                    if (sum[q].cur_sp >= 0) {
                        sp = sum[q].cur_sp;
                        break;
                    }
                }
            }
            st.ev_sp = sp;
        }
    }
    if (done && end < nseg && (sum[end].flags & SRE_SUM_ERROR)) st.error = 1;
    return st;
}

__global__ __launch_bounds__(64) void
sre_k_verify_c(sre_scan_tables_t T, sre_scan_geom_t G, const sre_seg_summary_t *__restrict__ sum,
               VerifyAcc *__restrict__ accs, sre_stream_status_t *__restrict__ status)
{
    SRE_TAIL_PRIO();
    const uint32_t s = blockIdx.x * blockDim.x + threadIdx.x;
    const bool     valid = s < G.nstreams;
    const uint32_t lane = threadIdx.x & 63u;
    sre_stream_status_t st;
    uint64_t            first = 0;
    st.ev_sp = -1;
    st.ev_seg = -1;
    if (valid) {
        const VerifyAcc acc = accs[s];
        accs[s].bad = accs[s].end = ~0ull;
        accs[s].count = accs[s].evseg = accs[s].spseg = accs[s].unst = accs[s].unst_end = 0;
        first = geom_first(G, s);
        const uint64_t nseg = geom_first(G, s + 1) - first;
        st = assemble_status(T, sum + first, nseg, acc, true);
    }
    uint64_t need = __builtin_amdgcn_ballot_w64(valid && st.ev_sp == SRE_EV_SP_SEARCH);
    while (need) {
        const int      l = __builtin_ctzll(need);
        need &= need - 1;
        const uint64_t f = __shfl(first, l, 64);
        const int64_t  top = __shfl(st.ev_seg, l, 64) - 1;
        int64_t        sp = 0;
        bool           found = false;
        for (int64_t hi = top; hi >= 0 && !found; hi -= 256) {
            int64_t v[4];
#pragma unroll
            for (int j = 0; j < 4; j++) {
                const int64_t q = hi - (int64_t) lane - 64 * j;
                v[j] = q >= 0 ? sum[f + (uint64_t) q].cur_sp : (int64_t) -1;
            }
#pragma unroll
            for (int j = 0; j < 4; j++) {
                const uint64_t b = __builtin_amdgcn_ballot_w64(v[j] >= 0);
                if (!found && b) {
                    sp = __shfl(v[j], __builtin_ctzll(b), 64);
                    found = true;
                }
            }
        }
        if ((int) lane == l) st.ev_sp = sp;
    }
    if (valid) status[s] = st;
}

#define SRE_VERIFY_ONE_MAX SRE_VERIFY_ONE_SEGS

template <int NT>
__device__ void
verify_one_stream(const sre_scan_tables_t &T, const sre_seg_summary_t *__restrict__ sum, uint64_t nseg,
                  sre_stream_status_t *__restrict__ status, VerifyAcc *sh_acc, sre_stream_status_t *out,
                  const sre_seg_digest_t *__restrict__ dig = nullptr)
{
    constexpr int  PER = SRE_VERIFY_ONE_MAX / NT;
    const uint32_t tid = threadIdx.x;
    if (tid == 0) {
        sh_acc->bad = sh_acc->end = ~0ull;
        sh_acc->count = sh_acc->evseg = sh_acc->spseg = sh_acc->unst = sh_acc->unst_end = 0;
    }
    uint32_t bits[PER], cnt[PER];
#pragma unroll
    for (int i = 0; i < PER; i++) {
        const uint64_t k = (uint64_t) i * NT + tid;
        bits[i] = 0;
        cnt[i] = 0;
        if (k < nseg && dig != nullptr) {
            const sre_seg_digest_t c = dig[k];
            const uint32_t         prev_out = k > 0 ? dig[k - 1].s_out : c.s_in;
            bits[i] = ((c.s_in == 0xffffffffu || c.s_in != prev_out) ? 1u : 0u) | c.bits;
            cnt[i] = c.count;
        } else if (k < nseg) {
            const sre_seg_summary_t &c = sum[k];
            const uint32_t s_in = c.s_in, fl = c.flags;
            const uint32_t prev_out = k > 0 ? sum[k - 1].s_out : s_in;
            bits[i] = ((s_in == 0xffffffffu || s_in != prev_out) ? 1u : 0u) | ((fl & SRE_SUM_TERM) ? 2u : 0u)
                      | ((fl & SRE_SUM_LASTEV) ? 4u : 0u) | (c.cur_sp >= 0 ? 8u : 0u) | ((fl & SRE_SUM_STABLE) ? 0u : 16u);
            cnt[i] = (uint32_t) c.count;
        }
    }
    __syncthreads();
    {
        unsigned long long bad = ~0ull, end = ~0ull;
#pragma unroll
        for (int i = PER - 1; i >= 0; i--) {
            const uint64_t k = (uint64_t) i * NT + tid;
            if (bits[i] & 1u) bad = k;
            if (bits[i] & 2u) end = k;
        }
        for (int d = 32; d >= 1; d >>= 1) {
            const unsigned long long b2 = __shfl_down(bad, d, 64), e2 = __shfl_down(end, d, 64);
            bad = b2 < bad ? b2 : bad;
            end = e2 < end ? e2 : end;
        }
        if ((tid & 63u) == 0) {
            if (bad != ~0ull) atomicMin(&sh_acc->bad, bad);
            if (end != ~0ull) atomicMin(&sh_acc->end, end);
        }
    }
    __syncthreads();
    {
        uint64_t bad = sh_acc->bad, end = sh_acc->end;
        if (bad > nseg) bad = nseg;
        if (end > nseg) end = nseg;
        const uint64_t     limit = end < bad ? end + 1 : bad;
        unsigned long long c = 0, ev = 0, sp = 0;
#pragma unroll
        for (int i = 0; i < PER; i++) {
            const uint64_t k = (uint64_t) i * NT + tid;
            if (k < limit) {
                c += cnt[i];
                if (bits[i] & 4u) ev = k + 1;
                if (bits[i] & 8u) sp = k + 1;
            }
        }
        for (int d = 32; d >= 1; d >>= 1) {
            c += __shfl_down(c, d, 64);
            const unsigned long long e2 = __shfl_down(ev, d, 64), s2 = __shfl_down(sp, d, 64);
            ev = e2 > ev ? e2 : ev;
            sp = s2 > sp ? s2 : sp;
        }
        if ((tid & 63u) == 0) {
            if (c) atomicAdd(&sh_acc->count, c);
            if (ev) atomicMax(&sh_acc->evseg, ev);
            if (sp) atomicMax(&sh_acc->spseg, sp);
        }
    }
    __syncthreads();
    {
// ... 518 lines not shown
        }
        if (p == tr.sp) {
            t = &L_trans[(size_t) nstates * nsym + variant];
            val = tr.sp;
        } else {
            const uint32_t s_prev = tr.state_before(p - 1);
            t = &L_trans[(size_t) s_prev * nsym + tr.sym_at(p - 1)];
            val = p;
        }
        const uint32_t lin = t->lin_off + j;
        const uint64_t m = L_lin_saves[lin] & unresolved;
        if (m) {
            for (uint32_t q = 0; q < nslots; q++) {
                if ((m >> q) & 1) vec[q] = val + base;
            }
            unresolved &= ~m;
        }
        if (lin_early != nullptr) {
            const uint64_t m2 = lin_early[lin] & unresolved;
            for (uint32_t q = 0; q < nslots; q++) {
                if ((m2 >> q) & 1) vec[q] = val - 1 + base;
            }
            unresolved &= ~m2;
        }
        if (p == tr.sp) break;
        j = L_lin_parent[lin];
        if (j == 0xffu) break;
#ifdef SRE_DEBUG_WALK
        tr.dbg_rest += wall_clock64() - dbg_c;
#endif
    }

        return 0;
    }
};

__device__ inline void
stage_walk_tables(const sre_scan_tables_t *__restrict__ tabp, uint8_t *lds, sre_scan_tables_t *Tsp)
{
    sre_scan_tables_t &Ts = *Tsp;
    {
        uint32_t *fast = reinterpret_cast<uint32_t *>(lds);
        uint8_t  *clsl = lds + tabp->fast_bytes;
        uint8_t  *trl = clsl + 256;
        const uint32_t tr_bytes = (tabp->nstates * (tabp->ncls + 1) + SRE_SCAN_NINIT) * (uint32_t) sizeof(sre_dev_trans_t);
        uint64_t *savl = reinterpret_cast<uint64_t *>(trl + tr_bytes);
        uint32_t *lofl = reinterpret_cast<uint32_t *>(savl + tabp->lin_total);
        uint32_t *lpcl = lofl + tabp->nstates + 1;
        uint8_t  *parl = reinterpret_cast<uint8_t *>(lpcl + tabp->list_total);
        if (threadIdx.x == 0) {
            Ts = *tabp;
            Ts.fast = fast;
            Ts.cls = clsl;
            Ts.trans = reinterpret_cast<const sre_dev_trans_t *>(trl);
            Ts.lin_saves = savl;
            Ts.lin_parent = parl;
            Ts.list_off = lofl;
            Ts.list_pcs = lpcl;
        }
        for (uint32_t i = threadIdx.x; i <= tabp->nstates; i += blockDim.x) lofl[i] = tabp->list_off[i];
        for (uint32_t i = threadIdx.x; i < tabp->list_total; i += blockDim.x) lpcl[i] = tabp->list_pcs[i];
        for (uint32_t i = threadIdx.x; i < tabp->lin_total; i += blockDim.x) {
            savl[i] = tabp->lin_saves[i];
            parl[i] = tabp->lin_parent[i];
        }
        for (uint32_t i = threadIdx.x; i < tabp->fast_bytes / 16; i += blockDim.x) {
            reinterpret_cast<uint4 *>(fast)[i] = reinterpret_cast<const uint4 *>(tabp->fast_plain)[i];
        }
        for (uint32_t i = threadIdx.x; i < tr_bytes / 8; i += blockDim.x) {
            reinterpret_cast<uint64_t *>(trl)[i] = reinterpret_cast<const uint64_t *>(tabp->trans)[i];
        }
        for (uint32_t i = threadIdx.x; i < 256; i += blockDim.x) clsl[i] = tabp->cls[i];
        __syncthreads();
    }
}

template <int NT>
__global__ __launch_bounds__(NT) void
sre_k_captures(const sre_scan_tables_t *__restrict__ tabp, sre_scan_geom_t G,
               const sre_seg_summary_t *__restrict__ sum,
               sre_stream_status_t *__restrict__ status, uint16_t *__restrict__ scratch,
               int64_t *__restrict__ records, uint32_t ovec_slots,
               const sre_seg_lineage_t *__restrict__ maps,
               const sre_seg_lineage_t *__restrict__ blocks, int use_maps)
{
    SRE_TAIL_PRIO();
    extern __shared__ __attribute__((aligned(16))) uint8_t lds[];
    __shared__ sre_scan_tables_t Ts;
    __shared__ uint16_t sh_trace[64][72];
    __shared__ uint8_t  sh_syms[64][72];
#ifdef SRE_DEBUG_WALK
    const unsigned long long dbg_t0 = wall_clock64();
#endif
    stage_walk_tables(tabp, lds, &Ts);
    if (NT != 64) {
        __shared__ VerifyAcc sh_acc;
        __shared__ sre_stream_status_t sh_st;
        verify_one_stream<NT>(Ts, sum, geom_first(G, 1), status, &sh_acc, &sh_st, G.digest);
    }
    const bool     lane_mode = NT == 64 && G.nstreams >= SRE_CAPTURE_LANE_STREAMS;
    if (!lane_mode && threadIdx.x != 0) return;
    const uint32_t wl = lane_mode ? threadIdx.x : 0u;
    auto one_stream = [&](const uint32_t s) {
    if (use_maps && !status[s].need_maps) return;
#ifdef SRE_DEBUG_WALK
    const unsigned long long dbg_ts = wall_clock64();
    unsigned long long       dbg_tw0 = 0, dbg_tw1 = 0;
#endif
    const sre_scan_tables_t   &T = Ts;
    const sre_stream_status_t  st = status[s];
    int64_t                   *rec = records + (size_t) s * (2 + ovec_slots);
    const uint32_t             nsym = T.ncls + 1;

    status[s].need_maps = 0;
    rec[0] = st.rc;
    rec[1] = st.count;
    for (uint32_t q = 0; q < ovec_slots; q++) rec[2 + q] = -1;
    if (!st.done) {
        rec[0] = RC_ERROR;
        return;
    }
    if (st.error && T.mode == SRE_HIP_PIKE_COUNT) rec[0] = RC_ERROR;
    if (st.ev_pos < 0) return;
    if (T.mode == 0) {
        rec[0] = 0;
        return;
    }

    Tracer tr;
    tr.T = &T;
    tr.sum = sum + geom_first(G, s);
    tr.data = geom_ptr(G, s);
    tr.n = (int64_t) geom_len(G, s);
    tr.sp = st.ev_sp;
    tr.seg_bytes = G.seg_bytes;
    const uint32_t variant = st.ev_sp == 0 ? G.init_variant : restart_variant(T, tr.data, st.ev_sp);
    tr.init_state = T.init[variant];
    tr.apos = (st.ev_apos >= st.ev_sp) ? st.ev_apos : -1;
    tr.astate = st.ev_astate;
    tr.ck = scratch + (size_t) s * (G.seg_bytes + 16);
    tr.trace = (__attribute__((address_space(3))) uint16_t *) sh_trace[wl];
    tr.syms = (__attribute__((address_space(3))) uint8_t *) sh_syms[wl];
    tr.bind();
    tr.seg_lo = tr.seg_hi = -1;
    tr.blk_lo = 1;
    tr.blk_hi = 0;
    tr.seg_entry = 0;
    tr.valid_from = first_valid_segment(tr.sum, tr.sp, (int64_t) G.seg_bytes, st.ev_seg);
    tr.use_stable = (T.mode == 1 && T.nshadow != 0);
    status[s].valid_from = (uint32_t) tr.valid_from;

    int64_t  vec[64];
    uint64_t unresolved = T.nslots >= 64 ? ~0ull : ((1ull << T.nslots) - 1);
    for (uint32_t q = 0; q < T.nslots; q++) vec[q] = -1;

    const sre_dev_trans_t &te = T.trans[(size_t) st.ev_state * nsym + st.ev_sym];
    uint32_t               j = te.src;
    if (te.kind == EV_DONE || te.kind == SRE_DEV_EV_DONE_EMPTY) {
        const uint64_t m = te.saves & unresolved;
        for (uint32_t q = 0; q < T.nslots; q++) {
            if ((m >> q) & 1) vec[q] = st.ev_pos + 1;
        }
        unresolved &= ~m;
    }
    if (te.early & unresolved) {
        const uint64_t m = te.early & unresolved;
        for (uint32_t q = 0; q < T.nslots; q++) {
            if ((m >> q) & 1) vec[q] = st.ev_pos;
        }
        unresolved &= ~m;
    }

    {
        LineageWalk lw;
        lw.T = &T;
        lw.tabp = tabp;
        lw.tr = &tr;
        lw.variant = variant;
        lw.ev_seg = st.ev_seg;
        lw.unst_seg = st.unst_seg;
        lw.unst_end = (int64_t) 1 << 62;
        lw.first = geom_first(G, s);
        lw.maps = maps;
        lw.blocks = blocks;
        lw.use_maps = use_maps != 0;
        lw.carried = nullptr;
        lw.carried_stride = 0;
        lw.base = 0;
        lw.walk_budget = SRE_WALK_BUDGET;
#ifdef SRE_DEBUG_WALK
        dbg_tw0 = wall_clock64();
#endif
        const int need = lw.run(st.ev_pos, j, st.ev_state, unresolved, vec);
#ifdef SRE_DEBUG_WALK
        dbg_tw1 = wall_clock64();
#endif
        if (need) {
            status[s].need_maps = 1;
            return;
        }
    }

    uint64_t ofs = 0;
    for (int64_t i = 0; i < st.rc; i++) ofs += T.multi_ncaps[i] + 1;
    ofs *= 2;
    const uint64_t ncopy = 2ull * (T.multi_ncaps[st.rc] + 1);
    for (uint64_t q = 0; q < ovec_slots; q++) rec[2 + q] = q < ncopy ? vec[ofs + q] : -1;
    rec[0] = (st.error && T.mode == SRE_HIP_PIKE_COUNT) ? RC_ERROR : st.rc;
#ifdef SRE_DEBUG_WALK
    printf("captures: stream %u (10 ns ticks) staging %llu, to the walk %llu, walk %llu, rest %llu; steps %u, load_segment %u calls %llu ticks "
           "(entry_state %llu), run_block %u calls %llu ticks; per step: top %llu, state_before(p) %llu, rest %llu\n", s,
           dbg_ts - dbg_t0, dbg_tw0 - dbg_ts, dbg_tw1 - dbg_tw0, wall_clock64() - dbg_tw1, tr.dbg_steps, tr.dbg_seg_calls,
           tr.dbg_seg_ticks, tr.dbg_entry_ticks, tr.dbg_blk_calls, tr.dbg_blk_ticks, tr.dbg_top, tr.dbg_sb, tr.dbg_rest);
#endif
    };
    if (lane_mode) {
        for (uint32_t s = blockIdx.x * 64u + wl; s < G.nstreams; s += gridDim.x * 64u) one_stream(s);
    } else {
        for (uint32_t s = blockIdx.x; s < G.nstreams; s += gridDim.x) one_stream(s);
    }
}


#define SRE_TAIL_THREADS 1024

struct TailCtxCompat {
    sre_stream_ctx_t *c;
    __device__ __forceinline__ uint32_t &state() const { return c->state; }
    __device__ __forceinline__ uint32_t &has_pending() const { return c->has_pending; }
    __device__ __forceinline__ int64_t  &pending_regex() const { return c->pending_regex; }
    __device__ __forceinline__ int64_t  *pending_vec() const { return c->pending_vec; }
    __device__ __forceinline__ int64_t  *caps() const { return &c->caps[0][0]; }
    __device__ __forceinline__ int64_t  *caps_next() const { return &c->caps_next[0][0]; }
    __device__ __forceinline__ uint32_t  stride() const { return SRE_STREAM_MAX_SLOTS; }
};
struct TailCtxRow {
    int64_t *row;
    uint32_t nslots, max_threads;
    __device__ __forceinline__ uint32_t &state() const { return reinterpret_cast<uint32_t *>(row + SRE_SROW_STATE)[0]; }
    __device__ __forceinline__ uint32_t &has_pending() const { return reinterpret_cast<uint32_t *>(row + SRE_SROW_STATE)[1]; }
    __device__ __forceinline__ int64_t  &pending_regex() const { return row[SRE_SROW_REGEX]; }
    __device__ __forceinline__ int64_t  *pending_vec() const { return row + SRE_SROW_HDR; }
    __device__ __forceinline__ int64_t  *caps() const { return row + SRE_SROW_HDR + nslots; }
    __device__ __forceinline__ int64_t  *caps_next() const { return row + SRE_SROW_HDR + nslots + (size_t) max_threads * nslots; }
    __device__ __forceinline__ uint32_t  stride() const { return nslots; }
};
struct TailChunk {
    const uint8_t           *data;
    int64_t                  n, base;
    const sre_seg_summary_t *sum;
    uint64_t                 nseg;
    uint32_t                 seg_bytes, variant, entry_state, ovec_slots;
    bool                     continues, eof;
    uint16_t                *scratch;
    __attribute__((address_space(3))) uint16_t *sh_trace;
    __attribute__((address_space(3))) uint8_t  *sh_syms;
};

template <class Ctx>
__device__ __forceinline__ int64_t
stream_tail_body(const sre_scan_tables_t &T, const sre_scan_tables_t *__restrict__ tabp, const sre_stream_status_t &st,
                 const TailChunk &K, const Ctx &ctx, sre_stream_result_t *__restrict__ res)
{
    int64_t                  rc_out = RC_ERROR;
    const sre_seg_summary_t *sum = K.sum;
    const uint64_t           nseg = K.nseg;
    const int64_t            base = K.base;
    const bool               eof = K.eof;
    const uint32_t           ovec_slots = K.ovec_slots;
    const uint32_t           nsym = T.ncls + 1;
    const bool               continues = K.continues;
    const int64_t            n = K.n;

    res->has_pending = 0;
    res->ev_in_chunk = 0;
    res->ev_slot1 = -1;
    res->poisoned = 0;
    res->next_state = 0;
    if (!continues) ctx.has_pending() = 0;
    if (!st.done) {
        rc_out = SRE_STREAM_UNSETTLED;
        return rc_out;
    }
    if (T.mode == 0) {
        const bool carried_match = continues && ctx.has_pending() != 0;
        bool       match_now = false, match_waits = false;
        if (carried_match) {
            match_now = n > 0 || eof;
            match_waits = !match_now;
        } else if (st.ev_pos >= 0) {
            const uint32_t kind = T.trans[(size_t) st.ev_state * (T.ncls + 1) + st.ev_sym].kind;
            const bool     listed_behind = (kind == EV_DONE || kind == SRE_DEV_EV_DONE_EMPTY);
            match_waits = listed_behind && st.ev_pos == n - 1 && !eof;
            match_now = !match_waits;
        }
        if (match_now) {
            rc_out = 0;
            ctx.state() = 0;
            ctx.has_pending() = 0;
        } else if (match_waits) {
            ctx.has_pending() = 1;
            ctx.state() = 1;
// ... 302 lines not shown
    return h_tab->any_fresh ? scan_kernel_bits<SRE_HIP_PIKE_COUNT, true>(h_tab->class_bits, h_tab->wide != 0)
                            : scan_kernel_bits<SRE_HIP_PIKE_COUNT, false>(h_tab->class_bits, h_tab->wide != 0);
}

extern "C" size_t
sre_scan_lds_bytes(const sre_scan_tables_t *h_tab)
{
    const size_t tr = ((size_t) h_tab->nstates * (h_tab->ncls + 1) * 2 + 15) & ~(size_t) 15;
    const size_t half = (size_t) SRE_SCAN_ROUND * h_tab->class_bits / 8 * (h_tab->wide ? 2 : 1);
    static const char *pad_env = getenv("SRE_HIP_LDS_PAD");
    const size_t pad = pad_env ? (size_t) atoi(pad_env) : 0;
    size_t       need = pad + (size_t) h_tab->fast_rows * SRE_FAST_ROW_BYTES + 256 + tr + ((h_tab->nstates + 15u) & ~15u)
                        + 16 + (size_t) SRE_SCAN_BLOCK * (2 * half + 16);
    return need + (size_t) SRE_SCAN_BLOCK * 16;
}

extern "C" int
sre_scan_blocks_per_cu(const sre_scan_tables_t *h_tab)
{
    int          n = 0;
    const size_t shmem = sre_scan_lds_bytes(h_tab);
    hipError_t   e;
    e = hipOccupancyMaxActiveBlocksPerMultiprocessor(&n, scan_kernel(h_tab), SRE_SCAN_BLOCK, shmem);
    if (e != hipSuccess || n < 1) n = 1;
    if (n > 8) n = 8;
    return n;
}

extern "C" hipError_t
sre_launch_scan(const sre_scan_tables_t *d_tab, sre_scan_tables_t h_tab, sre_scan_geom_t geom,
                sre_seg_summary_t *d_sum, const sre_stream_status_t *d_lo, const uint8_t *d_entry,
                hipStream_t stream)
{
    if (geom.nsegs == 0) return hipSuccess;
    const uint32_t grid = (uint32_t) ((geom.nsegs + SRE_SCAN_BLOCK - 1) / SRE_SCAN_BLOCK);
    const size_t   shmem = sre_scan_lds_bytes(&h_tab);
    if (shmem > 48 * 1024) {
        static bool raised[2][9][2];
        bool       &done = raised[h_tab.mode == SRE_HIP_PIKE_COUNT][h_tab.class_bits & 8 ? 8 : h_tab.class_bits][h_tab.wide != 0];
        if (!done) {
            hipError_t e = hipFuncSetAttribute(reinterpret_cast<const void *>(scan_kernel(&h_tab)),
                                               hipFuncAttributeMaxDynamicSharedMemorySize,
                                               SRE_SCAN_LDS_LIMIT);
            if (e != hipSuccess) return e;
            done = true;
        }
    }
    hipLaunchKernelGGL(scan_kernel(&h_tab), dim3(grid), dim3(SRE_SCAN_BLOCK), shmem, stream,
                       d_tab, geom, d_sum, d_lo, d_entry);
    return hipGetLastError();
}

__global__ __launch_bounds__(256) void
sre_k_upload_words(const uint64_t *__restrict__ src, uint64_t *__restrict__ dst, uint32_t n)
{
    for (uint32_t i = blockIdx.x * 256u + threadIdx.x; i < n; i += gridDim.x * 256u) dst[i] = src[i];
}

extern "C" hipError_t
sre_launch_upload_words(const uint64_t *h_src_mapped, uint64_t *d_dst, uint32_t nwords, hipStream_t stream)
{
    if (nwords == 0) return hipSuccess;
    const uint32_t grid = (nwords + 255) / 256 < 64 ? (nwords + 255) / 256 : 64;
    hipLaunchKernelGGL(sre_k_upload_words, dim3(grid), dim3(256), 0, stream, h_src_mapped, d_dst, nwords);
    return hipGetLastError();
}

extern "C" size_t
sre_scan_verify_acc_bytes(uint32_t nstreams)
{
    return (size_t) nstreams * sizeof(VerifyAcc);
}

extern "C" hipError_t
sre_scan_verify_acc_init(void *d_acc, uint32_t nstreams, hipStream_t stream)
{
    hipError_t e = hipMemset2DAsync(d_acc, sizeof(VerifyAcc), 0xff, 2 * sizeof(unsigned long long),
                                    nstreams, stream);
    if (e != hipSuccess) return e;
    return hipMemset2DAsync(static_cast<char *>(d_acc) + 2 * sizeof(unsigned long long),
                            sizeof(VerifyAcc), 0, 5 * sizeof(unsigned long long), nstreams, stream);
}

extern "C" hipError_t
sre_launch_verify(sre_scan_tables_t h_tab, sre_scan_geom_t geom, const sre_seg_summary_t *d_sum,
                  void *d_acc, sre_stream_status_t *d_status, hipStream_t stream)
{
    if (geom.nstreams == 0) return hipSuccess;
    VerifyAcc *acc = static_cast<VerifyAcc *>(d_acc);
    const uint32_t gseg = (uint32_t) ((geom.nsegs + 255) / 256);
    hipLaunchKernelGGL(sre_k_verify_a, dim3(gseg), dim3(256), 0, stream, geom, d_sum, acc, (int) h_tab.mode);
    const uint32_t gseg4 = (uint32_t) ((geom.nsegs + SRE_VERIFY_SPAN - 1) / SRE_VERIFY_SPAN);
    hipLaunchKernelGGL(sre_k_verify_b, dim3(gseg4), dim3(256), 0, stream, geom, d_sum, acc);
    if (h_tab.mode == 1  && h_tab.nshadow) {
        hipLaunchKernelGGL(sre_k_verify_b2, dim3(gseg4), dim3(256), 0, stream, geom, d_sum, acc);
    }
    hipLaunchKernelGGL(sre_k_verify_c, dim3((geom.nstreams + 63) / 64), dim3(64), 0, stream, h_tab,
                       geom, d_sum, acc, d_status);
    return hipGetLastError();
}

extern "C" hipError_t
sre_launch_captures(const sre_scan_tables_t *d_tab, sre_scan_tables_t h_tab, sre_scan_geom_t geom,
                    const sre_seg_summary_t *d_sum, sre_stream_status_t *d_status,
                    uint16_t *d_scratch, int64_t *d_records, uint32_t ovec_slots,
                    const sre_seg_lineage_t *d_maps, const sre_seg_lineage_t *d_blocks,
                    int use_maps, int verify, hipStream_t stream)
{
    if (geom.nstreams == 0) return hipSuccess;
    if (verify && (geom.nstreams != 1 || geom.nsegs > SRE_VERIFY_ONE_SEGS || h_tab.mode == SRE_HIP_PIKE_COUNT || use_maps)) {
        return hipErrorInvalidValue;
    }
    const uint32_t block = verify ? 1024 : 64;
    const uint32_t want = (!verify && geom.nstreams >= SRE_CAPTURE_LANE_STREAMS) ? (geom.nstreams + 63u) / 64u : geom.nstreams;
    const uint32_t grid = want < SRE_CAPTURE_MAX_GRID ? want : SRE_CAPTURE_MAX_GRID;
    const size_t   shmem = (size_t) h_tab.fast_bytes + 256
                         + ((size_t) h_tab.nstates * (h_tab.ncls + 1) + SRE_SCAN_NINIT) * sizeof(sre_dev_trans_t)
                         + (size_t) h_tab.lin_total * 9 + ((size_t) h_tab.nstates + 1 + h_tab.list_total) * 4 + 16;
    if (shmem > 48 * 1024) {
        static bool raised[2];
        if (!raised[verify != 0]) {
            hipError_t e = hipFuncSetAttribute(verify ? reinterpret_cast<const void *>(sre_k_captures<1024>)
                                                      : reinterpret_cast<const void *>(sre_k_captures<64>),
                                               hipFuncAttributeMaxDynamicSharedMemorySize, SRE_CAPTURE_LDS_LIMIT);
            if (e != hipSuccess) return e;
            raised[verify != 0] = true;
        }
    }
    if (verify) {
        hipLaunchKernelGGL(sre_k_captures<1024>, dim3(1), dim3(1024), shmem, stream, d_tab, geom, d_sum,
                           d_status, d_scratch, d_records, ovec_slots, d_maps, d_blocks, use_maps);
    } else {
        hipLaunchKernelGGL(sre_k_captures<64>, dim3(grid), dim3(block), shmem, stream, d_tab, geom, d_sum,
                           d_status, d_scratch, d_records, ovec_slots, d_maps, d_blocks, use_maps);
    }
    return hipGetLastError();
}

extern "C" hipError_t
sre_launch_lineage(const sre_scan_tables_t *d_tab, sre_scan_tables_t h_tab, sre_scan_geom_t geom,
                   const sre_seg_summary_t *d_sum, const sre_stream_status_t *d_status,
                   sre_seg_lineage_t *d_maps, sre_seg_lineage_t *d_blocks, hipStream_t stream)
{
    if (geom.nsegs == 0) return hipSuccess;
    const uint32_t nsym = h_tab.ncls + 1;
    const size_t   shmem = 256 + (size_t) h_tab.nstates * nsym * sizeof(sre_dev_trans_t)
                         + 2 * (size_t) ((h_tab.lin_total + 15u) & ~15u);
    const uint32_t gseg = (uint32_t) ((geom.nsegs + 255) / 256);
    if (shmem > 48 * 1024) {
        static bool raised = false;
        if (!raised) {
            hipError_t e = hipFuncSetAttribute(reinterpret_cast<const void *>(sre_k_lineage_maps),
                                               hipFuncAttributeMaxDynamicSharedMemorySize, SRE_CAPTURE_LDS_LIMIT);
            if (e != hipSuccess) return e;
            raised = true;
        }
    }
    hipLaunchKernelGGL(sre_k_lineage_maps, dim3(gseg), dim3(256), shmem, stream, d_tab, geom, d_sum,
                       d_status, d_maps);
    const uint64_t nblocks = geom.nsegs / SRE_LINEAGE_BLOCK;
    if (nblocks) {
        hipLaunchKernelGGL(sre_k_lineage_blocks, dim3((uint32_t) ((nblocks * 16 + 255) / 256)), dim3(256), 0,
                           stream, geom.nsegs, d_maps, d_blocks);
    }
    return hipGetLastError();
}

extern "C" hipError_t
sre_launch_exact_entries(const sre_scan_tables_t *d_tab, sre_scan_tables_t h_tab, sre_scan_geom_t geom,
                         const sre_seg_summary_t *d_sum, const sre_stream_status_t *d_status,
                         uint8_t *d_fn, uint8_t *d_comp, uint8_t *d_chunk_entry, uint8_t *d_entry,
                         hipStream_t stream)
{
    if (geom.nsegs == 0) return hipSuccess;
    const uint64_t nchunks = (geom.nsegs + SRE_FN_CHUNK - 1) / SRE_FN_CHUNK;
    hipError_t     e;
    if ((e = hipMemsetAsync(d_entry, 0xff, geom.nsegs, stream)) != hipSuccess) return e;
    if ((e = hipMemsetAsync(d_chunk_entry, 0xff, nchunks, stream)) != hipSuccess) return e;
    const size_t shmem = (size_t) (h_tab.nstates + 1) * SRE_FAST_ROW_BYTES + 256
                         + (((size_t) h_tab.nstates * (h_tab.ncls + 1) * 2 + 15) & ~(size_t) 15);
    const uint32_t grid = (uint32_t) ((geom.nsegs + 3) / 4);
    void (*kern)(const sre_scan_tables_t *, sre_scan_geom_t, const sre_stream_status_t *, uint8_t *) =
        h_tab.class_bits == 1 ? sre_k_seg_functions<1> : h_tab.class_bits == 2 ? sre_k_seg_functions<2>
        : h_tab.class_bits == 4 ? sre_k_seg_functions<4> : sre_k_seg_functions<8>;
    if (shmem > 48 * 1024) {
        e = hipFuncSetAttribute(reinterpret_cast<const void *>(kern), hipFuncAttributeMaxDynamicSharedMemorySize,
                                (int) shmem);
        if (e != hipSuccess) return e;
    }
    hipLaunchKernelGGL(kern, dim3(grid), dim3(256), shmem, stream, d_tab, geom, d_status, d_fn);
    hipLaunchKernelGGL(sre_k_fn_chunks, dim3((uint32_t) nchunks), dim3(64), 0, stream, geom.nsegs, d_fn, d_comp);
    hipLaunchKernelGGL(sre_k_fn_resolve, dim3((geom.nstreams + 63) / 64), dim3(64), 0, stream, geom, d_sum,
                       d_status, d_fn, d_comp, d_entry, d_chunk_entry);
    hipLaunchKernelGGL(sre_k_fn_fill, dim3((uint32_t) ((nchunks + 63) / 64)), dim3(64), 0, stream, geom.nsegs,
                       d_fn, d_chunk_entry, d_entry);
    return hipGetLastError();
}

extern "C" hipError_t
sre_launch_stream_tail(const sre_scan_tables_t *d_tab, sre_scan_tables_t h_tab, sre_scan_geom_t geom,
                       const sre_seg_summary_t *d_sum, sre_stream_status_t *d_status,
                       uint16_t *d_scratch, sre_stream_ctx_t *d_ctx, sre_stream_result_t *result, int64_t base,
                       int eof, uint32_t ovec_slots, int verify, hipStream_t stream)
{
    const size_t shmem = (size_t) h_tab.fast_bytes + 256
                         + ((size_t) h_tab.nstates * (h_tab.ncls + 1) + SRE_SCAN_NINIT) * sizeof(sre_dev_trans_t)
                         + (size_t) h_tab.lin_total * 9 + ((size_t) h_tab.nstates + 1 + h_tab.list_total) * 4 + 16;
    if (shmem > 48 * 1024) {
        static bool raised = false;
        if (!raised) {
            hipError_t e = hipFuncSetAttribute(reinterpret_cast<const void *>(sre_k_stream_tail),
                                               hipFuncAttributeMaxDynamicSharedMemorySize, SRE_CAPTURE_LDS_LIMIT);
            if (e != hipSuccess) return e;
            raised = true;
        }
    }
    hipLaunchKernelGGL(sre_k_stream_tail, dim3(1), dim3(SRE_TAIL_THREADS), shmem, stream, d_tab, geom, d_sum, d_status,
// ... 28 lines not shown
```

Measured before the change: 6137 GB/s.

## Replace atomic verify passes with span-reduction kernel, fused combine and direct host publish

For multi-segment scans the old verify used several atomic passes (verify_a/b/b2/c) over segment summaries. These are replaced by a per-span associative reduction over segment digests, using wave shuffles in one kernel. The per-stream combine step is deferred into the captures kernel, which also writes records and status straight to pinned host memory and so skips the final device-to-host copy. This cuts kernel launches and atomics on the tail of each job, in exchange for extra digest and span buffers and more complex merge semantics.

New measurement: 6168 GB/s (median of 6 runs). About the same (+0.5%).

```diff
diff --git a/sregex_amd/csrc/sre_hip_batch.cpp b/sregex_amd/csrc/sre_hip_batch.cpp
--- a/sregex_amd/csrc/sre_hip_batch.cpp
+++ b/sregex_amd/csrc/sre_hip_batch.cpp
@@ -1,6 +1,7 @@
 #include <sregex_hip.h>
 #include "sre_hip_runtime.h"
 #include "sre_hip_scan.h"
+#include "sre_verify_span.h"
 #include "sre_scan_host.h"
 #include "sre_dfa.h"
 #include "sre_nfa.h"
@@ -55,9 +56,11 @@
     uint64_t                  seg_cap_env;
     sre_scan_geom_t           geom;
     uint64_t                 *d_seg_first, *h_seg_first;
+    uint64_t                 *d_span_first, *h_span_first;
     sre_seg_summary_t        *d_sum;
     sre_seg_digest_t         *d_digest;
-    size_t                    sum_cap;
+    sre_verify_span_t        *d_spans;
+    size_t                    sum_cap, digest_cap, spans_cap;
     sre_stream_status_t      *d_status, *h_status;
     void                     *d_acc;
     int64_t                  *d_lo, *h_lo;
@@ -206,6 +209,7 @@
     if (sc->d_ctx) (void) hipFree(sc->d_ctx);
     if (sc->d_sum) (void) hipFree(sc->d_sum);
     if (sc->d_digest) (void) hipFree(sc->d_digest);
+    if (sc->d_spans) (void) hipFree(sc->d_spans);
     if (sc->d_acc) (void) hipFree(sc->d_acc);
     if (sc->d_lo) (void) hipFree(sc->d_lo);
     if (sc->h_lo) (void) hipHostFree(sc->h_lo);
@@ -732,7 +736,7 @@
         sc->d_acc = NULL;
         sc->d_lo = sc->h_lo = NULL;
         sc->cap_streams = 0;
-        const size_t in_bytes = (3 * n + 1) * sizeof(uint64_t);
+        const size_t in_bytes = (4 * n + 2) * sizeof(uint64_t);
         const size_t out_bytes = record_bytes(sc, n) + n * sizeof(sre_stream_status_t);
         static_assert(sizeof(sre_nfa_status_t) <= sizeof(sre_stream_status_t), "status block");
         static_assert(sizeof(sre_nfa_status_t) == sizeof(sre_nfa_window_t), "window layout");
@@ -757,9 +761,11 @@
     sc->h_ptrs = reinterpret_cast<const void **>(sc->h_in);
     sc->h_lens = sc->h_in + n;
     sc->h_seg_first = sc->h_in + 2 * n;
+    sc->h_span_first = sc->h_in + 3 * n + 1;
     sc->d_ptrs = reinterpret_cast<const void **>(sc->d_in);
     sc->d_lens = sc->d_in + n;
     sc->d_seg_first = sc->d_in + 2 * n;
+    sc->d_span_first = sc->d_in + 3 * n + 1;
     sc->d_records = reinterpret_cast<sre_int_t *>(sc->d_out);
     sc->h_records = reinterpret_cast<sre_int_t *>(sc->h_out);
     sc->d_status = reinterpret_cast<sre_stream_status_t *>(sc->d_out + record_bytes(sc, n));
@@ -861,7 +867,7 @@
     return (uint64_t) sre_hip_cu_count() * (uint64_t) sc->blocks_per_cu * SRE_SCAN_BLOCK;
 }
 
-static int scan_buffers(sre_hip_scanner_t *sc, size_t nstreams, uint64_t seg, uint64_t nsegs);
+static int scan_buffers(sre_hip_scanner_t *sc, size_t nstreams, uint64_t seg, uint64_t nsegs, uint64_t nspans);
 
 static int
 nfa_buffers(sre_hip_scanner_t *sc, uint64_t nsegs)
@@ -897,13 +903,16 @@
         const uint64_t resident = scan_resident(sc);
         seg = sre_scan_auto_segment(total, resident, scan_seg_cap(sc));
     }
-    uint64_t nsegs = 0;
+    uint64_t nsegs = 0, nspans = 0;
     for (size_t i = 0; i < nstreams; i++) {
         sc->h_seg_first[i] = nsegs;
+        sc->h_span_first[i] = nspans;
         uint64_t k = (sc->h_lens[i] + seg - 1) / seg;
         nsegs += k ? k : 1;
+        nspans += sre_vspan_count(k ? k : 1);
     }
     sc->h_seg_first[nstreams] = nsegs;
+    sc->h_span_first[nstreams] = nspans;
     geom_clear(sc);
     sc->geom.streams = reinterpret_cast<const uint8_t *const *>(sc->d_ptrs);
     sc->geom.lens = sc->d_lens;
@@ -918,11 +927,11 @@
     sc->geom.flags = flags | ((nstreams == 1 && sc->engine == SRE_HIP_ENGINE_SCAN) ? SRE_GEOM_ONE : 0u);
 
     if (sc->engine == SRE_HIP_ENGINE_NFA) return nfa_buffers(sc, nsegs);
-    return scan_buffers(sc, nstreams, seg, nsegs);
-}
-
-static int
-scan_buffers(sre_hip_scanner_t *sc, size_t nstreams, uint64_t seg, uint64_t nsegs)
+    return scan_buffers(sc, nstreams, seg, nsegs, nspans);
+}
+
+static int
+scan_buffers(sre_hip_scanner_t *sc, size_t nstreams, uint64_t seg, uint64_t nsegs, uint64_t nspans)
 {
     if (nsegs > sc->sum_cap) {
         if (sc->d_sum) (void) hipFree(sc->d_sum);
@@ -932,13 +941,31 @@
         sc->sum_cap = nsegs;
     }
     sc->geom.digest = NULL;
-    if (nsegs <= SRE_VERIFY_ONE_SEGS && sc->mode != SRE_HIP_PIKE_COUNT) {
-        if (sc->d_digest == NULL
-            && hipMalloc(reinterpret_cast<void **>(&sc->d_digest), SRE_VERIFY_ONE_SEGS * sizeof(sre_seg_digest_t)) != hipSuccess)
-        {
+    sc->geom.spans = NULL;
+    sc->geom.span_first = NULL;
+    sc->geom.nspans = 0;
+    if ((nsegs <= SRE_VERIFY_ONE_SEGS || nspans != 0) && sc->mode != SRE_HIP_PIKE_COUNT) {
+        if (nsegs > sc->digest_cap) {
+            const size_t want = nsegs > SRE_VERIFY_ONE_SEGS ? nsegs : SRE_VERIFY_ONE_SEGS;
+            if (sc->d_digest) (void) hipFree(sc->d_digest);
             sc->d_digest = NULL;
+            sc->digest_cap = 0;
+            if (hipMalloc(reinterpret_cast<void **>(&sc->d_digest), want * sizeof(sre_seg_digest_t)) == hipSuccess) sc->digest_cap = want;
+            else sc->d_digest = NULL;
         }
         sc->geom.digest = sc->d_digest;
+        if (nspans > sc->spans_cap) {
+            if (sc->d_spans) (void) hipFree(sc->d_spans);
+            sc->d_spans = NULL;
+            sc->spans_cap = 0;
+            if (hipMalloc(reinterpret_cast<void **>(&sc->d_spans), nspans * sizeof(sre_verify_span_t)) == hipSuccess) sc->spans_cap = nspans;
+            else sc->d_spans = NULL;
+        }
+        if (nspans != 0 && sc->d_digest != NULL && sc->d_spans != NULL) {
+            sc->geom.spans = sc->d_spans;
+            sc->geom.span_first = sc->d_span_first;
+            sc->geom.nspans = nspans;
+        }
     }
     {
         size_t need = nstreams * ((size_t) seg + 16);
@@ -1247,6 +1274,7 @@
 {
     hipStream_t    stream = static_cast<hipStream_t>(hip_stream);
     const uint32_t init_variant = sc->next_init_variant;
+    bool           published = false;
     call_begin(sc);
     sc->next_init_variant = 0;
     if (nstreams == 0) {
@@ -1297,10 +1325,10 @@
         if (!one) {
             static const bool dma = getenv("SRE_HIP_DMA_UPLOAD") != NULL;
             if (dma) {
-                SRE_HIP_TRY(hipMemcpyAsync(sc->d_in, sc->h_in, (3 * nstreams + 1) * sizeof(uint64_t),
+                SRE_HIP_TRY(hipMemcpyAsync(sc->d_in, sc->h_in, (4 * nstreams + 2) * sizeof(uint64_t),
                                            hipMemcpyHostToDevice, stream));
             } else {
-                SRE_HIP_TRY(sre_launch_upload_words(sc->h_in, sc->d_in, (uint32_t) (3 * nstreams + 1), stream));
+                SRE_HIP_TRY(sre_launch_upload_words(sc->h_in, sc->d_in, (uint32_t) (4 * nstreams + 2), stream));
             }
         }
         if (scan_events(sc) != 0) return -1;
@@ -1314,16 +1342,21 @@
         }
         {
             const int fused = one && sc->geom.nsegs <= SRE_VERIFY_ONE_SEGS && sc->mode != SRE_HIP_PIKE_COUNT;
-            if (!fused) SRE_HIP_TRY(sre_launch_verify(sc->tab->h, sc->geom, sc->d_sum, sc->d_acc, sc->d_status, stream));
-            SRE_HIP_TRY(sre_launch_captures(sc->tab->d_tab, sc->tab->h, sc->geom, sc->d_sum, sc->d_status,
-                                            sc->d_scratch, sc->d_records, sc->ovec_slots,
-                                            NULL, NULL, 0, fused, stream));
-        }
-    }
-    SRE_HIP_TRY(hipMemcpyAsync(sc->h_out, sc->d_out,
-                               record_bytes(sc, nstreams)
-                                   + (sc->engine != SRE_HIP_ENGINE_VM ? nstreams * sizeof(sre_stream_status_t) : 0),
-                               hipMemcpyDeviceToHost, stream));
+            const int combine = !fused && sre_verify_defers_combine(sc->tab->h, sc->geom);
+            if (!fused) SRE_HIP_TRY(sre_launch_verify(sc->tab->h, sc->geom, sc->d_sum, sc->d_acc, sc->d_status, combine, stream));
+            published = nstreams < SRE_CAPTURE_LANE_STREAMS;
+            SRE_HIP_TRY(sre_launch_captures_publish(sc->tab->d_tab, sc->tab->h, sc->geom, sc->d_sum, sc->d_status,
+                                                    sc->d_scratch, sc->d_records, sc->ovec_slots,
+                                                    NULL, NULL, 0, combine ? 2 : fused, published ? sc->h_records : NULL,
+                                                    published ? sc->h_status : NULL, stream));
+        }
+    }
+    if (!published) {
+        SRE_HIP_TRY(hipMemcpyAsync(sc->h_out, sc->d_out,
+                                   record_bytes(sc, nstreams)
+                                       + (sc->engine != SRE_HIP_ENGINE_VM ? nstreams * sizeof(sre_stream_status_t) : 0),
+                                   hipMemcpyDeviceToHost, stream));
+    }
     if (sc->ev_done == NULL) SRE_HIP_TRY(hipEventCreateWithFlags(&sc->ev_done, hipEventDisableTiming));
     SRE_HIP_TRY(hipEventRecord(sc->ev_done, stream));
     sc->last_n = nstreams;
@@ -1399,7 +1432,7 @@
                 sc->exact_passes++;
             }
             SRE_HIP_TRY(sre_launch_scan(sc->tab->d_tab, sc->tab->h, sc->geom, sc->d_sum, sc->d_status, d_entry, stream));
-            SRE_HIP_TRY(sre_launch_verify(sc->tab->h, sc->geom, sc->d_sum, sc->d_acc, sc->d_status, stream));
+            SRE_HIP_TRY(sre_launch_verify(sc->tab->h, sc->geom, sc->d_sum, sc->d_acc, sc->d_status, 0, stream));
             if (with_captures) {
                 SRE_HIP_TRY(sre_launch_captures(sc->tab->d_tab, sc->tab->h, sc->geom, sc->d_sum,
                                                 sc->d_status, sc->d_scratch, sc->d_records,
@@ -1725,11 +1758,11 @@
         const uint64_t i1 = sc->h_linfo->i1, nb = i1 - i0, seg = sc->h_linfo->seg, nsegs = sc->h_linfo->nsegs;
         call_begin(sc);
         geom_device(sc, nb, seg, nsegs);
-        if (scan_buffers(sc, nb, seg, nsegs) != 0) return -1;
+        if (scan_buffers(sc, nb, seg, nsegs, 0) != 0) return -1;
         SRE_HIP_TRY(hipEventRecord(sc->ev0, stream));
         SRE_HIP_TRY(sre_launch_scan(sc->tab->d_tab, sc->tab->h, sc->geom, sc->d_sum, NULL, NULL, stream));
         SRE_HIP_TRY(hipEventRecord(sc->ev1, stream));
-        SRE_HIP_TRY(sre_launch_verify(sc->tab->h, sc->geom, sc->d_sum, sc->d_acc, sc->d_status, stream));
+        SRE_HIP_TRY(sre_launch_verify(sc->tab->h, sc->geom, sc->d_sum, sc->d_acc, sc->d_status, 0, stream));
         SRE_HIP_TRY(sre_launch_captures(sc->tab->d_tab, sc->tab->h, sc->geom, sc->d_sum, sc->d_status,
                                         sc->d_scratch, sc->d_records, sc->ovec_slots, NULL, NULL, 0, 0, stream));
         if (lines_status_counters(sc, nb, stream) != 0) return -1;
@@ -3334,7 +3367,7 @@
     SRE_HIP_TRY(sre_launch_scan(sc->tab->d_tab, sc->tab->h, sc->geom, sc->d_sum, NULL, NULL, stream));
     {
         const int fused = sc->geom.nsegs <= SRE_VERIFY_ONE_SEGS;
-        if (!fused) SRE_HIP_TRY(sre_launch_verify(sc->tab->h, sc->geom, sc->d_sum, sc->d_acc, sc->d_status, stream));
+        if (!fused) SRE_HIP_TRY(sre_launch_verify(sc->tab->h, sc->geom, sc->d_sum, sc->d_acc, sc->d_status, 0, stream));
         SRE_HIP_TRY(sre_launch_stream_tail(sc->tab->d_tab, sc->tab->h, sc->geom, sc->d_sum, sc->d_status,
                                            sc->d_scratch, d_ctx, d_res, base, eof, ovec_slots, fused, stream));
     }
@@ -3690,11 +3723,11 @@
     if (h_info->nsegs != 0) {
         const uint64_t seg = h_info->seg, nsegs = h_info->nsegs;
         const uint32_t grid = streams_tail_grid(h_info->nactive);
-        if (scan_buffers(sc, grid, seg, nsegs) != 0) return -1;
+        if (scan_buffers(sc, grid, seg, nsegs, 0) != 0) return -1;
         geom_device(sc, n, seg, nsegs);
         sc->geom.sentry = ss->d_sentry;
         SRE_HIP_TRY(sre_launch_scan(sc->tab->d_tab, sc->tab->h, sc->geom, sc->d_sum, NULL, NULL, stream));
-        SRE_HIP_TRY(sre_launch_verify(sc->tab->h, sc->geom, sc->d_sum, sc->d_acc, sc->d_status, stream));
+        SRE_HIP_TRY(sre_launch_verify(sc->tab->h, sc->geom, sc->d_sum, sc->d_acc, sc->d_status, 0, stream));
         SRE_HIP_TRY(sre_launch_streams_tail(sc->tab->d_tab, sc->tab->h, sc->geom, sc->d_sum, sc->d_status, sc->d_scratch,
                                             ss->d_rows, ss->L, ss->d_tailres, d_recs, d_info, grid, 0, stream));
         ss->launches += 1 + (sc->mode == SRE_HIP_PIKE_FIRST && sc->tab->h.nshadow ? 4 : 3) + 1;
diff --git a/sregex_amd/csrc/sre_hip_scan.h b/sregex_amd/csrc/sre_hip_scan.h
--- a/sregex_amd/csrc/sre_hip_scan.h
+++ b/sregex_amd/csrc/sre_hip_scan.h
@@ -168,6 +168,9 @@
     uint64_t one_len;
     const uint8_t *sflags;
     struct sre_seg_digest_s *digest;
+    struct sre_verify_span_t *spans;
+    const uint64_t *span_first;
+    uint64_t nspans;
     const uint32_t *sentry;
 } sre_scan_geom_t;
 #define SRE_SENTRY_STATE(e)   ((e) & 0xffffu)
@@ -238,14 +241,20 @@
 hipError_t sre_launch_upload_words(const uint64_t *h_src_mapped, uint64_t *d_dst, uint32_t nwords, hipStream_t stream);
 size_t sre_scan_verify_acc_bytes(uint32_t nstreams);
 hipError_t sre_scan_verify_acc_init(void *d_acc, uint32_t nstreams, hipStream_t stream);
+int sre_verify_defers_combine(sre_scan_tables_t h_tab, sre_scan_geom_t geom);
 hipError_t sre_launch_verify(sre_scan_tables_t h_tab, sre_scan_geom_t geom,
     const sre_seg_summary_t *d_sum, void *d_acc, sre_stream_status_t *d_status,
-    hipStream_t stream);
+    int defer_combine, hipStream_t stream);
 hipError_t sre_launch_captures(const sre_scan_tables_t *d_tab, sre_scan_tables_t h_tab,
     sre_scan_geom_t geom, const sre_seg_summary_t *d_sum, sre_stream_status_t *d_status,
     uint16_t *d_scratch, int64_t *d_records, uint32_t ovec_slots,
     const sre_seg_lineage_t *d_maps, const sre_seg_lineage_t *d_blocks, int use_maps,
     int verify, hipStream_t stream);
+hipError_t sre_launch_captures_publish(const sre_scan_tables_t *d_tab, sre_scan_tables_t h_tab,
+    sre_scan_geom_t geom, const sre_seg_summary_t *d_sum, sre_stream_status_t *d_status,
+    uint16_t *d_scratch, int64_t *d_records, uint32_t ovec_slots,
+    const sre_seg_lineage_t *d_maps, const sre_seg_lineage_t *d_blocks, int use_maps,
+    int verify, int64_t *h_records, sre_stream_status_t *h_status, hipStream_t stream);
 hipError_t sre_launch_lineage(const sre_scan_tables_t *d_tab, sre_scan_tables_t h_tab,
     sre_scan_geom_t geom, const sre_seg_summary_t *d_sum, const sre_stream_status_t *d_status,
     sre_seg_lineage_t *d_maps, sre_seg_lineage_t *d_blocks, hipStream_t stream);
diff --git a/sregex_amd/csrc/sre_hip_scan.hip b/sregex_amd/csrc/sre_hip_scan.hip
--- a/sregex_amd/csrc/sre_hip_scan.hip
+++ b/sregex_amd/csrc/sre_hip_scan.hip
@@ -3,6 +3,7 @@
 #include "sre_hip_scan.h"
 #include "sre_hip_streams.h"
 #include "sre_hip_tile.h"
+#include "sre_verify_span.h"
 
 #define SRE_HIP_PIKE_COUNT 2
 #define EV_DONE 1
@@ -1206,12 +1207,7 @@
 }
 
 
-struct VerifyAcc {
-    unsigned long long bad, end;
-    unsigned long long count, evseg, spseg;
-    unsigned long long unst;
-    unsigned long long unst_end;
-};
+typedef sre_verify_acc_t VerifyAcc;
 
 __global__ __launch_bounds__(256) void
 sre_k_verify_a(sre_scan_geom_t G, const sre_seg_summary_t *__restrict__ sum, VerifyAcc *__restrict__ acc,
@@ -1253,7 +1249,6 @@
     if (ke != ~0ull && ke < __hip_atomic_load(&acc[s].end, __ATOMIC_RELAXED, __HIP_MEMORY_SCOPE_AGENT)) atomicMin(&acc[s].end, ke);
 }
 
-#define SRE_VERIFY_SPAN 1024u
 
 __global__ __launch_bounds__(256) void
 sre_k_verify_b(sre_scan_geom_t G, const sre_seg_summary_t *__restrict__ sum, VerifyAcc *__restrict__ acc)
@@ -1478,6 +1473,104 @@
     if (valid) status[s] = st;
 }
 
+static_assert(SRE_VERIFY_SPAN == 4 * 256, "sre_k_verify_spans: four segments per thread");
+
+__device__ inline sre_verify_span_t
+vspan_wave_fold(sre_verify_span_t r)
+{
+    const uint32_t lane = threadIdx.x & 63u;
+    for (int d = 1; d < 64; d <<= 1) {
+        sre_verify_span_t o;
+        o.bad = __shfl_down(r.bad, d, 64);
+        o.term = __shfl_down(r.term, d, 64);
+        o.count = __shfl_down(r.count, d, 64);
+        o.ev = __shfl_down(r.ev, d, 64);
+        o.sp = __shfl_down(r.sp, d, 64);
+        o.unst_all = __shfl_down(r.unst_all, d, 64);
+        o.unst_ev = __shfl_down(r.unst_ev, d, 64);
+        o.unst_in = __shfl_down(r.unst_in, d, 64);
+        if (lane + (uint32_t) d < 64u) r = sre_vspan_merge(r, o);
+    }
+    return r;
+}
+
+__device__ inline uint32_t
+vspan_stream_of(const sre_scan_geom_t &G, uint64_t p)
+{
+    if (G.flags & SRE_GEOM_ONE) return 0;
+    uint32_t a = 0, b = G.nstreams;
+    while (b - a > 1) {
+        uint32_t m = (a + b) >> 1;
+        if (G.span_first[m] <= p) a = m; else b = m;
+    }
+    return a;
+}
+
+__global__ __launch_bounds__(256) void
+sre_k_verify_spans(sre_scan_geom_t G)
+{
+    SRE_TAIL_PRIO();
+    __shared__ sre_verify_span_t sh[4];
+    const uint64_t p = blockIdx.x;
+    if (p >= G.nspans) return;
+    const uint32_t s = vspan_stream_of(G, p);
+    const uint64_t first = geom_first(G, s), nseg = geom_first(G, s + 1) - first;
+    const uint64_t j = p - ((G.flags & SRE_GEOM_ONE) ? 0 : G.span_first[s]);
+    const sre_seg_digest_t *__restrict__ dig = G.digest + first;
+    sre_verify_span_t r = sre_vspan_none();
+    const uint64_t    k0 = j * SRE_VERIFY_SPAN + 4u * threadIdx.x;
+    if (k0 < nseg) {
+        sre_seg_digest_t c[4];
+        uint32_t         prev_out = 0;
+#pragma unroll
+        for (int i = 0; i < 4; i++) {
+            c[i].s_in = c[i].s_out = c[i].bits = c[i].count = 0;
+            if (k0 + i < nseg) c[i] = dig[k0 + i];
+        }
+        if (k0 > 0) prev_out = dig[k0 - 1].s_out;
+#pragma unroll
+        for (int i = 0; i < 4; i++) {
+            if (k0 + i < nseg) r = sre_vspan_merge(r, sre_vspan_one(k0 + i, nseg, c[i].s_in, prev_out, c[i].bits, c[i].count));
+            prev_out = c[i].s_out;
+        }
+    }
+    r = vspan_wave_fold(r);
+    if ((threadIdx.x & 63u) == 0) sh[threadIdx.x >> 6] = r;
+    __syncthreads();
+    if (threadIdx.x == 0) {
+        r = sh[0];
+        for (int w = 1; w < 4; w++) r = sre_vspan_merge(r, sh[w]);
+        G.spans[p] = r;
+    }
+}
+
+__device__ inline void
+verify_combine_stream(const sre_scan_tables_t &T, const sre_scan_geom_t &G, const sre_seg_summary_t *__restrict__ sum,
+                      sre_stream_status_t *__restrict__ status, uint32_t s)
+{
+    const uint32_t lane = threadIdx.x & 63u;
+    const bool     unst = T.mode == 1  && T.nshadow != 0;
+    const uint64_t first = geom_first(G, s), nseg = geom_first(G, s + 1) - first;
+    const uint64_t p0 = (G.flags & SRE_GEOM_ONE) ? 0 : G.span_first[s];
+    const uint64_t n = sre_vspan_count(nseg);
+    sre_verify_span_t acc = sre_vspan_none();
+    for (uint64_t j0 = 0; j0 < n; j0 += 64) {
+        sre_verify_span_t r = sre_vspan_none();
+        if (j0 + lane < n) r = G.spans[p0 + j0 + lane];
+        acc = sre_vspan_merge(acc, vspan_wave_fold(r));
+    }
+    if (lane == 0) status[s] = assemble_status(T, sum + first, nseg, sre_vspan_acc(acc, unst), true);
+}
+
+__global__ __launch_bounds__(256) void
+sre_k_verify_combine(sre_scan_tables_t T, sre_scan_geom_t G, const sre_seg_summary_t *__restrict__ sum,
+                     sre_stream_status_t *__restrict__ status)
+{
+    SRE_TAIL_PRIO();
+    const uint32_t s = blockIdx.x * 4u + (threadIdx.x >> 6);
+    if (s < G.nstreams) verify_combine_stream(T, G, sum, status, s);
+}
+
 #define SRE_VERIFY_ONE_MAX SRE_VERIFY_ONE_SEGS
 
 template <int NT>
@@ -2162,7 +2255,8 @@
                sre_stream_status_t *__restrict__ status, uint16_t *__restrict__ scratch,
                int64_t *__restrict__ records, uint32_t ovec_slots,
                const sre_seg_lineage_t *__restrict__ maps,
-               const sre_seg_lineage_t *__restrict__ blocks, int use_maps)
+               const sre_seg_lineage_t *__restrict__ blocks, int use_maps, int combine,
+               int64_t *__restrict__ h_records, sre_stream_status_t *__restrict__ h_status)
 {
     SRE_TAIL_PRIO();
     extern __shared__ __attribute__((aligned(16))) uint8_t lds[];
@@ -2177,6 +2271,9 @@
         __shared__ VerifyAcc sh_acc;
         __shared__ sre_stream_status_t sh_st;
         verify_one_stream<NT>(Ts, sum, geom_first(G, 1), status, &sh_acc, &sh_st, G.digest);
+    }
+    if (NT == 64 && combine) {
+        for (uint32_t s = blockIdx.x; s < G.nstreams; s += gridDim.x) verify_combine_stream(Ts, G, sum, status, s);
     }
     const bool     lane_mode = NT == 64 && G.nstreams >= SRE_CAPTURE_LANE_STREAMS;
     if (!lane_mode && threadIdx.x != 0) return;
@@ -2294,10 +2391,22 @@
            tr.dbg_seg_ticks, tr.dbg_entry_ticks, tr.dbg_blk_calls, tr.dbg_blk_ticks, tr.dbg_top, tr.dbg_sb, tr.dbg_rest);
 #endif
     };
+    auto publish = [&](const uint32_t s) {
+        if (h_records == nullptr) return;
+        const size_t w = 2 + (size_t) ovec_slots;
+        for (size_t q = 0; q < w; q++) h_records[(size_t) s * w + q] = records[(size_t) s * w + q];
+        h_status[s] = status[s];
+    };
     if (lane_mode) {
-        for (uint32_t s = blockIdx.x * 64u + wl; s < G.nstreams; s += gridDim.x * 64u) one_stream(s);
+        for (uint32_t s = blockIdx.x * 64u + wl; s < G.nstreams; s += gridDim.x * 64u) {
+            one_stream(s);
+            publish(s);
+        }
     } else {
-        for (uint32_t s = blockIdx.x; s < G.nstreams; s += gridDim.x) one_stream(s);
+        for (uint32_t s = blockIdx.x; s < G.nstreams; s += gridDim.x) {
+            one_stream(s);
+            publish(s);
+        }
     }
 }
 
@@ -2766,11 +2875,32 @@
                             sizeof(VerifyAcc), 0, 5 * sizeof(unsigned long long), nstreams, stream);
 }
 
+static bool
+verify_by_spans(const sre_scan_tables_t &h_tab, const sre_scan_geom_t &geom)
+{
+    return h_tab.mode != SRE_HIP_PIKE_COUNT && geom.digest != nullptr && geom.spans != nullptr
+           && ((geom.flags & SRE_GEOM_ONE) || geom.span_first != nullptr);
+}
+
+extern "C" int
+sre_verify_defers_combine(sre_scan_tables_t h_tab, sre_scan_geom_t geom)
+{
+    return verify_by_spans(h_tab, geom) && geom.nstreams < SRE_CAPTURE_LANE_STREAMS;
+}
+
 extern "C" hipError_t
 sre_launch_verify(sre_scan_tables_t h_tab, sre_scan_geom_t geom, const sre_seg_summary_t *d_sum,
-                  void *d_acc, sre_stream_status_t *d_status, hipStream_t stream)
+                  void *d_acc, sre_stream_status_t *d_status, int defer_combine, hipStream_t stream)
 {
     if (geom.nstreams == 0) return hipSuccess;
+    if (verify_by_spans(h_tab, geom)) {
+        hipLaunchKernelGGL(sre_k_verify_spans, dim3((uint32_t) geom.nspans), dim3(256), 0, stream, geom);
+        if (!(defer_combine && sre_verify_defers_combine(h_tab, geom))) {
+            hipLaunchKernelGGL(sre_k_verify_combine, dim3((geom.nstreams + 3) / 4), dim3(256), 0, stream, h_tab, geom, d_sum,
+                               d_status);
+        }
+        return hipGetLastError();
+    }
     VerifyAcc *acc = static_cast<VerifyAcc *>(d_acc);
     const uint32_t gseg = (uint32_t) ((geom.nsegs + 255) / 256);
     hipLaunchKernelGGL(sre_k_verify_a, dim3(gseg), dim3(256), 0, stream, geom, d_sum, acc, (int) h_tab.mode);
@@ -2791,7 +2921,21 @@
                     const sre_seg_lineage_t *d_maps, const sre_seg_lineage_t *d_blocks,
                     int use_maps, int verify, hipStream_t stream)
 {
+    return sre_launch_captures_publish(d_tab, h_tab, geom, d_sum, d_status, d_scratch, d_records, ovec_slots, d_maps, d_blocks,
+                                       use_maps, verify, nullptr, nullptr, stream);
+}
+
+extern "C" hipError_t
+sre_launch_captures_publish(const sre_scan_tables_t *d_tab, sre_scan_tables_t h_tab, sre_scan_geom_t geom,
+                            const sre_seg_summary_t *d_sum, sre_stream_status_t *d_status,
+                            uint16_t *d_scratch, int64_t *d_records, uint32_t ovec_slots,
+                            const sre_seg_lineage_t *d_maps, const sre_seg_lineage_t *d_blocks,
+                            int use_maps, int verify, int64_t *h_records, sre_stream_status_t *h_status, hipStream_t stream)
+{
     if (geom.nstreams == 0) return hipSuccess;
+    const int combine = verify == 2;
+    if (combine && (!sre_verify_defers_combine(h_tab, geom) || use_maps)) return hipErrorInvalidValue;
+    if (combine) verify = 0;
     if (verify && (geom.nstreams != 1 || geom.nsegs > SRE_VERIFY_ONE_SEGS || h_tab.mode == SRE_HIP_PIKE_COUNT || use_maps)) {
         return hipErrorInvalidValue;
     }
@@ -2813,10 +2957,10 @@
     }
     if (verify) {
         hipLaunchKernelGGL(sre_k_captures<1024>, dim3(1), dim3(1024), shmem, stream, d_tab, geom, d_sum,
-                           d_status, d_scratch, d_records, ovec_slots, d_maps, d_blocks, use_maps);
+                           d_status, d_scratch, d_records, ovec_slots, d_maps, d_blocks, use_maps, 0, h_records, h_status);
     } else {
         hipLaunchKernelGGL(sre_k_captures<64>, dim3(grid), dim3(block), shmem, stream, d_tab, geom, d_sum,
-                           d_status, d_scratch, d_records, ovec_slots, d_maps, d_blocks, use_maps);
+                           d_status, d_scratch, d_records, ovec_slots, d_maps, d_blocks, use_maps, combine, h_records, h_status);
     }
     return hipGetLastError();
 }
diff --git a/sregex_amd/csrc/sre_verify_span.h b/sregex_amd/csrc/sre_verify_span.h
--- /dev/null
+++ b/sregex_amd/csrc/sre_verify_span.h
@@ -0,0 +1,98 @@
+#ifndef SRE_VERIFY_SPAN_H
+#define SRE_VERIFY_SPAN_H
+
+#include <stdint.h>
+
+#if defined(__HIPCC__)
+#define SRE_VSPAN_FN static __host__ __device__ inline
+#else
+#define SRE_VSPAN_FN static inline
+#endif
+
+#define SRE_VERIFY_SPAN 1024u
+#define SRE_VSPAN_NONE  (~0ull)
+
+#define SRE_DG_TERM     2u
+#define SRE_DG_LASTEV   4u
+#define SRE_DG_SP       8u
+#define SRE_DG_UNSTABLE 16u
+
+struct sre_verify_acc_t {
+    unsigned long long bad, end;
+    unsigned long long count, evseg, spseg;
+    unsigned long long unst;
+    unsigned long long unst_end;
+};
+
+struct sre_verify_span_t {
+    unsigned long long bad, term;
+    unsigned long long count, ev, sp;
+    unsigned long long unst_all, unst_ev, unst_in;
+};
+
+SRE_VSPAN_FN uint64_t
+sre_vspan_count(uint64_t nseg)
+{
+    return (nseg + SRE_VERIFY_SPAN - 1) / SRE_VERIFY_SPAN;
+}
+
+SRE_VSPAN_FN sre_verify_span_t
+sre_vspan_none(void)
+{
+    sre_verify_span_t r;
+    r.bad = r.term = SRE_VSPAN_NONE;
+    r.count = r.ev = r.sp = 0;
+    r.unst_all = r.unst_ev = r.unst_in = 0;
+    return r;
+}
+
+SRE_VSPAN_FN sre_verify_span_t
+sre_vspan_one(uint64_t k, uint64_t nseg, uint32_t s_in, uint32_t prev_out, uint32_t bits, uint32_t count)
+{
+    sre_verify_span_t r = sre_vspan_none();
+    const bool        broken = s_in == 0xffffffffu || (k > 0 && s_in != prev_out);
+    if (broken) r.bad = k;
+    if (bits & SRE_DG_TERM) r.term = k;
+    if (!broken) {
+        r.count = count;
+        if (bits & SRE_DG_LASTEV) r.ev = k + 1;
+        if (bits & SRE_DG_SP) r.sp = k + 1;
+    }
+    if (bits & SRE_DG_UNSTABLE) {
+        r.unst_all = k + 1;
+        if (k + 1 < nseg) r.unst_in = k + 1;
+    }
+    return r;
+}
+
+SRE_VSPAN_FN sre_verify_span_t
+sre_vspan_merge(const sre_verify_span_t &a, const sre_verify_span_t &b)
+{
+    sre_verify_span_t r;
+    const bool        stops = a.bad != SRE_VSPAN_NONE || a.term != SRE_VSPAN_NONE;
+    r.bad = a.bad != SRE_VSPAN_NONE ? a.bad : b.bad;
+    r.term = a.term != SRE_VSPAN_NONE ? a.term : b.term;
+    r.count = stops ? a.count : a.count + b.count;
+    r.ev = (stops || b.ev == 0) ? a.ev : b.ev;
+    r.sp = (stops || b.sp == 0) ? a.sp : b.sp;
+    r.unst_all = b.unst_all ? b.unst_all : a.unst_all;
+    r.unst_in = b.unst_in ? b.unst_in : a.unst_in;
+    r.unst_ev = (stops || b.ev == 0) ? a.unst_ev : (b.unst_ev ? b.unst_ev : a.unst_all);
+    return r;
+}
+
+SRE_VSPAN_FN sre_verify_acc_t
+sre_vspan_acc(const sre_verify_span_t &r, bool unst)
+{
+    sre_verify_acc_t acc;
+    acc.bad = r.bad;
+    acc.end = r.term;
+    acc.count = r.count;
+    acc.evseg = r.ev;
+    acc.spseg = r.sp;
+    acc.unst = unst ? r.unst_ev : 0;
+    acc.unst_end = unst ? r.unst_in : 0;
+    return acc;
+}
+
+#endif
```
